# a-to-the-5/Simple-MapReduce-Search-Engine-Information-Retrieval-

Measured on AMD Instinct MI355X. Metric: index build GB/s of text (top-10 queries/sec in 'query'), higher is better.
Workload: dtype u8 text / int32 postings / f64 weights

## Files before the change

simple-mapreduce-search-engine-information-retrieval-_amd/csrc/sme_build.hip:

```cpp
#include <hip/hip_runtime.h>
#include <limits.h>
#include <math.h>
#include <stdio.h>
#include <stdlib.h>
#include <string.h>

#include <algorithm>
#include <memory>
#include <chrono>

#include "sme_internal.hpp"
#include "sme_text.hpp"
#include "sme_trec.hpp"

namespace sme {


template <typename B>
__device__ bool doc_tag_valid(const B &t, int64_t p, const char *tag, int tl) {
  int chain = 0;
  int64_t x = p;
  for (;;) {
    int64_t q = -1;
    for (int j = 1; j < tl; j++) {
// ... 2490 lines not shown
                              uint32_t *ck) {
  for (int64_t i = blockIdx.x * (int64_t)blockDim.x + threadIdx.x; i < P; i += (int64_t)gridDim.x * blockDim.x)
    ck[i] = (key[i] << tfbits) | (tfmask - (uint32_t)tf[i]);
}
__global__ void k_composite32_tf(const uint32_t *ck, int64_t P, uint32_t tfmask, int32_t *tf) {
  for (int64_t i = blockIdx.x * (int64_t)blockDim.x + threadIdx.x; i < P; i += (int64_t)gridDim.x * blockDim.x)
    tf[i] = (int32_t)(tfmask - (ck[i] & tfmask));
}

__global__ void k_term_idf(const int64_t *off, int64_t V, double idf_ref, int64_t N, const int64_t *gdf,
                           const double *idf_by_df, int64_t sdf, const double *idf_by_q, int mode, double *idf) {
  for (int64_t t = blockIdx.x * (int64_t)blockDim.x + threadIdx.x; t < V; t += (int64_t)gridDim.x * blockDim.x) {
    if (mode == SME_IDF_REFERENCE) {
      idf[t] = idf_ref;
    } else {
      const int64_t df = gdf ? gdf[t] : off[t + 1] - off[t];
      idf[t] = df <= sdf ? idf_by_df[df] : idf_by_q[N / df];
    }
  }
}

__global__ void k_composite(const uint32_t *key, const int32_t *tf, int64_t P, int tfbits, uint64_t tfmask,
                            uint64_t *ck) {
  for (int64_t i = blockIdx.x * (int64_t)blockDim.x + threadIdx.x; i < P; i += (int64_t)gridDim.x * blockDim.x)
    ck[i] = ((uint64_t)key[i] << tfbits) | (tfmask - (uint64_t)tf[i]);
}
__global__ void k_composite_tf(const uint64_t *ck, int64_t P, uint64_t tfmask, int32_t *tf) {
  for (int64_t i = blockIdx.x * (int64_t)blockDim.x + threadIdx.x; i < P; i += (int64_t)gridDim.x * blockDim.x)
    tf[i] = (int32_t)(tfmask - (ck[i] & tfmask));
}

__global__ void k_docno_keys(const int32_t *docno, int64_t nR, uint32_t *k, uint32_t *v) {
  for (int64_t i = blockIdx.x * (int64_t)blockDim.x + threadIdx.x; i < nR; i += (int64_t)gridDim.x * blockDim.x) {
    k[i] = (uint32_t)docno[i] ^ 0x80000000u;
    v[i] = (uint32_t)i;
  }
}
__global__ void k_widen_u32(const uint32_t *a, int64_t n, int64_t *b) {
  for (int64_t i = blockIdx.x * (int64_t)blockDim.x + threadIdx.x; i < n; i += (int64_t)gridDim.x * blockDim.x)
    b[i] = (int64_t)a[i];
}
__global__ void k_not_ascending(const int32_t *d, int64_t n, unsigned long long *cnt) {
  bool bad = false;
  for (int64_t i = blockIdx.x * (int64_t)blockDim.x + threadIdx.x + 1; i < n; i += (int64_t)gridDim.x * blockDim.x)
    bad |= d[i] <= d[i - 1];
  if (__any(bad) && (threadIdx.x & 63) == 0) atomicAdd(cnt, 1ull);
}
__global__ void k_iota_i64(int64_t *a, int64_t n) {
  for (int64_t i = blockIdx.x * (int64_t)blockDim.x + threadIdx.x; i < n; i += (int64_t)gridDim.x * blockDim.x) a[i] = i;
}
__global__ void k_adjacent_equal(const uint32_t *k, int64_t n, unsigned long long *cnt) {
  for (int64_t i = blockIdx.x * (int64_t)blockDim.x + threadIdx.x + 1; i < n; i += (int64_t)gridDim.x * blockDim.x)
    if (k[i] == k[i - 1]) atomicAdd(cnt, 1ull);
}
__global__ void k_gather_i64(const int64_t *idx, int64_t n, const int32_t *src, int32_t *dst) {
  for (int64_t i = blockIdx.x * (int64_t)blockDim.x + threadIdx.x; i < n; i += (int64_t)gridDim.x * blockDim.x)
    dst[i] = src[idx[i]];
}
__global__ void k_fill_slow_lens(const int64_t *list, int64_t n, const uint64_t *rs, const uint64_t *re,
                                 int64_t *lens) {
  for (int64_t i = blockIdx.x * (int64_t)blockDim.x + threadIdx.x; i < n; i += (int64_t)gridDim.x * blockDim.x)
    lens[i] = (int64_t)(re[list[i]] - rs[list[i]]) + 1;
}
__global__ void k_compact_flags(const uint8_t *flag, int64_t n, int64_t *list, unsigned long long *cnt) {
  for (int64_t i = blockIdx.x * (int64_t)blockDim.x + threadIdx.x; i < n; i += (int64_t)gridDim.x * blockDim.x)
    if (flag[i]) list[atomicAdd(cnt, 1ull)] = i;
}
__global__ void k_long_lens(const int64_t *list, int64_t n, const int32_t *rlist, const unsigned long long *rep,
                            int64_t *lens) {
  for (int64_t i = blockIdx.x * (int64_t)blockDim.x + threadIdx.x; i < n; i += (int64_t)gridDim.x * blockDim.x) {
    uint32_t len = (uint32_t)(rep[rlist[list[i]]] & 0xFFFFFFull);
    asm volatile("" : "+v"(len));
    lens[i] = 5 * (int64_t)len + 32;
  }
}
__global__ void k_big_list(const int32_t *prec, int64_t n, int64_t *list, unsigned long long *cnt) {
  for (int64_t i = blockIdx.x * (int64_t)blockDim.x + threadIdx.x; i < n; i += (int64_t)gridDim.x * blockDim.x)
    if (prec[i] < 0) list[atomicAdd(cnt, 1ull)] = i;
}
__global__ void k_agg_regions(const int64_t *perm, const int32_t *ntok, int64_t nR, const int32_t *max_nout,
                              int64_t *reg, unsigned long long *mx) {
  unsigned long long m = 0;
  const int64_t mn = max(*max_nout, 1);
  for (int64_t i = blockIdx.x * (int64_t)blockDim.x + threadIdx.x; i < nR; i += (int64_t)gridDim.x * blockDim.x) {
    const int64_t c = (int64_t)ntok[perm[i]] * mn;
    reg[i] = c;
    m = max(m, (unsigned long long)c);
  }
  for (int o = 32; o > 0; o >>= 1) m = max(m, (unsigned long long)__shfl_xor(m, o, 64));
  if ((threadIdx.x & 63) == 0 && m) atomicMax(mx, m);
}
__global__ void k_big_caps(const int64_t *list, int64_t nbig, const int64_t *perm, const int32_t *ntok,
                           const int32_t *max_nout, int64_t *caps) {
  for (int64_t b = blockIdx.x * (int64_t)blockDim.x + threadIdx.x; b < nbig; b += (int64_t)gridDim.x * blockDim.x) {
    int64_t need = (int64_t)ntok[perm[list[b]]] * (int64_t)max(*max_nout, 1) * 2 + 64;
    int64_t c = 1;
    while (c < need) c <<= 1;
    caps[b] = c;
  }
}

__global__ void k_gather_u64(const uint64_t *src, const uint32_t *idx, int64_t nn, uint64_t *dst) {
  for (int64_t i = blockIdx.x * (int64_t)blockDim.x + threadIdx.x; i < nn; i += (int64_t)gridDim.x * blockDim.x)
    dst[i] = src[idx[i]];
}
__global__ void k_iota_u32(uint32_t *a, int64_t nn) {
  for (int64_t i = blockIdx.x * (int64_t)blockDim.x + threadIdx.x; i < nn; i += (int64_t)gridDim.x * blockDim.x)
    a[i] = (uint32_t)i;
}
__global__ void k_pair_counts(const int32_t *prec, const int32_t *bcount, int64_t n, int64_t *out) {
  for (int64_t i = blockIdx.x * (int64_t)blockDim.x + threadIdx.x; i < n; i += (int64_t)gridDim.x * blockDim.x)
    out[i] = prec[i] >= 0 ? prec[i] : bcount[i];
}

constexpr int kGCap = 1024;
constexpr int kGLimit = 768;

__device__ __forceinline__ int32_t nterms_of(const AggIn &in, uint32_t slot) {
  const int32_t rt = in.raw_term[slot];
  return rt >= 0 ? 1 : (rt <= -2 ? in.raw_nout[slot] : 0);
}

__global__ __launch_bounds__(kAggNT) void k_tcount(AggIn in, int64_t nR, int64_t *tcnt) {
  const int wv = threadIdx.x >> 6, lane = threadIdx.x & 63;
  const int64_t nwaves = (int64_t)gridDim.x * (kAggNT / 64);
  for (int64_t i = (int64_t)blockIdx.x * (kAggNT / 64) + wv; i < nR; i += nwaves) {
    const int64_t r = in.perm[i];
    const uint32_t *ts = in.tokstream + (in.rs[r] >> 1);
    const int32_t nt = in.ntok[r];
    int64_t c = 0;
    for (int32_t t = lane; t < nt; t += 64) c += nterms_of(in, ts[t]);
    for (int o = 32; o > 0; o >>= 1) c += __shfl_xor(c, o, 64);
    if (lane == 0) tcnt[i] = c;
  }
}

__global__ __launch_bounds__(kAggNT) void k_twrite(AggIn in, int64_t nR, const int64_t *toff, int32_t *tstream) {
  const int wv = threadIdx.x >> 6, lane = threadIdx.x & 63;
  const int64_t nwaves = (int64_t)gridDim.x * (kAggNT / 64);
  for (int64_t i = (int64_t)blockIdx.x * (kAggNT / 64) + wv; i < nR; i += nwaves) {
    const int64_t r = in.perm[i];
    const uint32_t *ts = in.tokstream + (in.rs[r] >> 1);
    const int32_t nt = in.ntok[r];
    int64_t o = toff[i];
    for (int32_t t0 = 0; t0 < nt; t0 += 64) {
      const int32_t t = t0 + lane;
      const uint32_t slot = t < nt ? ts[t] : 0u;
      const int32_t c = t < nt ? nterms_of(in, slot) : 0;
      const int32_t inc = wave_incl_sum(c);
      const int64_t at = o + inc - c;
      if (c == 1 && in.raw_term[slot] >= 0) {
        tstream[at] = in.raw_term[slot];
      } else if (c > 0) {
        const int32_t m0 = -in.raw_term[slot] - 2;
        for (int32_t m = 0; m < c; m++) tstream[at + m] = in.multi_term[m0 + m];
      }
      o += __shfl(inc, 63, 64);
    }
  }
}

__global__ void k_stream_to_merged(int32_t *tstream, int64_t M, const int64_t *wrank, const int64_t *drank) {
  for (int64_t i = blockIdx.x * (int64_t)blockDim.x + threadIdx.x; i < M; i += (int64_t)gridDim.x * blockDim.x) {
    const int32_t v = tstream[i];
    tstream[i] = (int32_t)((v & kDocCode) ? drank[v & ~kDocCode] : wrank[v]);
  }
}
__global__ void k_stream_docno(const int64_t *perm, const int32_t *docno, int64_t nR, int32_t *out) {
  for (int64_t i = blockIdx.x * (int64_t)blockDim.x + threadIdx.x; i < nR; i += (int64_t)gridDim.x * blockDim.x)
    out[i] = docno[perm[i]];
}

__device__ __forceinline__ uint64_t gram_key(const int32_t *ts, int K, int tb) {
  uint64_t k = 0;
  for (int j = 0; j < K; j++) k = (k << tb) | (uint64_t)(uint32_t)ts[j];
  return k;
}

__device__ __forceinline__ bool gram_insert(uint64_t *keys, int32_t *cnt, uint64_t key, int32_t *distinct) {
  uint32_t h = (uint32_t)fmix64(key) & (kGCap - 1);
  for (int probe = 0; probe < kGCap; probe++) {
    const unsigned long long old = atomicCAS((unsigned long long *)&keys[h], ~0ull, (unsigned long long)key);
    if (old == ~0ull) {
      atomicAdd(distinct, 1);
      atomicAdd(&cnt[h], 1);
      return true;
    }
    if (old == key) {
      atomicAdd(&cnt[h], 1);
      return true;
    }
    h = (h + 1) & (kGCap - 1);
  }
  return false;
}

template <bool EMIT>
__global__ __launch_bounds__(kAggNT) void k_gram_agg(const int32_t *tstream, const int64_t *toff, int64_t nR,
                                                     const int64_t *perm, const int32_t *docno_r, int K, int tb,
                                                     int64_t *pcount, uint8_t *big, const int64_t *pair_off,
                                                     uint64_t *pkey, uint64_t *pval, const uint32_t *pos_key) {
  __shared__ uint64_t keys_all[kAggNT / 64][kGCap];
  __shared__ int32_t cnt_all[kAggNT / 64][kGCap];
  __shared__ int32_t dist_all[kAggNT / 64];
  const int wv = threadIdx.x >> 6, lane = threadIdx.x & 63;
  uint64_t *keys = keys_all[wv];
  int32_t *cnt = cnt_all[wv];
  int32_t *distinct = &dist_all[wv];
  const int64_t nwaves = (int64_t)gridDim.x * (kAggNT / 64);
  for (int64_t i = (int64_t)blockIdx.x * (kAggNT / 64) + wv; i < nR; i += nwaves) {
    const int32_t *ts = tstream + toff[i];
    const int64_t m = toff[i + 1] - toff[i];
    const int64_t ng = m >= K ? m - K + 1 : 0;
    const uint64_t dn = (uint64_t)(uint32_t)docno_r[perm[i]] << 32;
    if (EMIT && big[i]) {
      for (int64_t j = lane; j < ng; j += 64) {
        pkey[pair_off[i] + j] = pos_key ? (uint64_t)pos_key[toff[i] + j] : gram_key(ts + j, K, tb);
        pval[pair_off[i] + j] = dn | 1u;
      }
      continue;
    }
    for (int k = lane; k < kGCap; k += 64) {
      keys[k] = ~0ull;
      cnt[k] = 0;
    }
    if (lane == 0) *distinct = 0;
    wave_sync_lds();
    bool ok = true;
    for (int64_t j = lane; j < ng; j += 64)
      ok &= gram_insert(keys, cnt, pos_key ? (uint64_t)pos_key[toff[i] + j] : gram_key(ts + j, K, tb), distinct);
    wave_sync_lds();
    const int32_t d = *distinct;
    const bool isbig = __any(!ok) || d > kGLimit;
    if (!EMIT) {
      if (lane == 0) {
        pcount[i] = isbig ? ng : d;
        big[i] = isbig;
      }
      wave_sync_lds();
      continue;
    }
    int64_t base = pair_off[i];
    for (int k = 0; k < kGCap / 64; k++) {
      const uint64_t key = keys[k * 64 + lane];
      const uint64_t mb = __ballot(key != ~0ull);
      if (key != ~0ull) {
        const int64_t o = base + __popcll(mb & ((1ull << lane) - 1ull));
        pkey[o] = key;
        pval[o] = dn | (uint32_t)cnt[k * 64 + lane];
      }
      base += __popcll(mb);
    }
    wave_sync_lds();
  }
}

__global__ void k_gram_flags(const uint64_t *k, int64_t P, uint32_t *f) {
  for (int64_t i = blockIdx.x * (int64_t)blockDim.x + threadIdx.x; i < P; i += (int64_t)gridDim.x * blockDim.x)
    f[i] = (i == 0 || k[i] != k[i - 1]) ? 1u : 0u;
}
__global__ void k_gram_ids(const uint64_t *k, const uint32_t *incl, int64_t P, int K, int tb, uint32_t *gid,
                           int32_t *gcomp) {
  for (int64_t i = blockIdx.x * (int64_t)blockDim.x + threadIdx.x; i < P; i += (int64_t)gridDim.x * blockDim.x) {
    const uint32_t g = incl[i] - 1;
    gid[i] = g;
    if (i == 0 || k[i] != k[i - 1])
      for (int j = 0; j < K; j++) gcomp[(int64_t)g * K + j] = (int32_t)((k[i] >> (tb * (K - 1 - j))) & ((1ull << tb) - 1));
  }
}

__global__ __launch_bounds__(kAggNT) void k_gram_round_keys(const int32_t *tstream, const int64_t *toff, int64_t nR,
                                                            int j, int tb, const uint32_t *rprev, uint64_t *key,
                                                            uint32_t *pos) {
  const int wv = threadIdx.x >> 6, lane = threadIdx.x & 63;
  const int64_t nwaves = (int64_t)gridDim.x * (kAggNT / 64);
  for (int64_t i = (int64_t)blockIdx.x * (kAggNT / 64) + wv; i < nR; i += nwaves) {
    const int64_t a = toff[i], e = toff[i + 1];
    for (int64_t p = a + lane; p < e; p += 64) {
      const bool valid = p + j - 1 < e;
      const uint64_t prev = rprev ? (uint64_t)rprev[p] : (uint64_t)(uint32_t)tstream[p];
      key[p] = valid ? (prev << tb) | (uint64_t)(uint32_t)tstream[p + j - 1] : ~0ull;
      pos[p] = (uint32_t)p;
    }
  }
}
__global__ void k_gram_round_heads(const uint64_t *ks, int64_t M, uint32_t *head) {
  for (int64_t s = blockIdx.x * (int64_t)blockDim.x + threadIdx.x; s < M; s += (int64_t)gridDim.x * blockDim.x)
    head[s] = (ks[s] != ~0ull && (s == 0 || ks[s] != ks[s - 1])) ? 1u : 0u;
}
__global__ void k_gram_round_scatter(const uint64_t *ks, const uint32_t *ps, const uint32_t *head,
                                     const uint32_t *excl, int64_t M, uint32_t *rnew, uint32_t *rep) {
  for (int64_t s = blockIdx.x * (int64_t)blockDim.x + threadIdx.x; s < M; s += (int64_t)gridDim.x * blockDim.x) {
    if (ks[s] == ~0ull) continue;
    const uint32_t r = excl[s] + head[s] - 1u;
    rnew[ps[s]] = r;
    if (rep && head[s]) rep[r] = ps[s];
  }
}
__global__ void k_gram_comp_rep(const uint32_t *rep, int64_t Vg, int K, const int32_t *tstream, int32_t *gcomp) {
  for (int64_t g = blockIdx.x * (int64_t)blockDim.x + threadIdx.x; g < Vg; g += (int64_t)gridDim.x * blockDim.x)
    for (int c = 0; c < K; c++) gcomp[g * K + c] = tstream[(int64_t)rep[g] + c];
}

constexpr int kTfTiny = 8;
constexpr int kTfSmall = 64;
constexpr int kTfWave = 512;
constexpr int kTfMedium = 8192;
constexpr int kTfSortMaxTf = 1023;

__global__ __launch_bounds__(256) void k_tfsort_tiny(const int64_t *__restrict__ off, int64_t V,
                                                     const int32_t *__restrict__ docno_d,
                                                     const int32_t *__restrict__ tf_d, int32_t *docno_o,
                                                     int32_t *tf_o) {
  for (int64_t s = blockIdx.x * (int64_t)blockDim.x + threadIdx.x; s < V; s += (int64_t)gridDim.x * blockDim.x) {
    const int64_t b = off[s];
    const int n = (int)(off[s + 1] - b);
    if (n > kTfTiny || n == 0) continue;
    int32_t t[kTfTiny], d[kTfTiny];
#pragma unroll
    for (int j = 0; j < kTfTiny; j++) {
      t[j] = j < n ? tf_d[b + j] : INT_MIN;
      d[j] = j < n ? docno_d[b + j] : 0;
    }
#pragma unroll
    for (int j = 1; j < kTfTiny; j++) {
#pragma unroll
      for (int k = j; k > 0; k--) {
        if (t[k - 1] < t[k]) {
          const int32_t x = t[k - 1], y = d[k - 1];
          t[k - 1] = t[k];
          d[k - 1] = d[k];
          t[k] = x;
          d[k] = y;
        }
      }
    }
#pragma unroll
    for (int j = 0; j < kTfTiny; j++)
      if (j < n) {
        docno_o[b + j] = d[j];
        tf_o[b + j] = t[j];
      }
  }
}

__global__ __launch_bounds__(256) void k_tfsort_small(const int64_t *__restrict__ off,
                                                      const int32_t *__restrict__ seg,
                                                      const unsigned long long *__restrict__ nseg,
                                                      const int32_t *__restrict__ docno_d,
                                                      const int32_t *__restrict__ tf_d, int32_t *docno_o,
                                                      int32_t *tf_o) {
  const int lane = threadIdx.x & 63;
  const int64_t nw = (int64_t)gridDim.x * (blockDim.x >> 6), ns = (int64_t)*nseg;
  for (int64_t q = (int64_t)blockIdx.x * (blockDim.x >> 6) + (threadIdx.x >> 6); q < ns; q += nw) {
    const int64_t s = seg[q];
    const int64_t b = off[s];
    const int n = (int)(off[s + 1] - b);
    const bool v = lane < n;
    const int32_t t = v ? tf_d[b + lane] : 0, d = v ? docno_d[b + lane] : 0;
    int r = 0;
    for (int j = 0; j < n; j++) {
      const int32_t tj = __shfl(t, j, 64);
      r += (tj > t) || (tj == t && j < lane);
    }
    if (v) {
      docno_o[b + r] = d;
      tf_o[b + r] = t;
    }
  }
}

template <int NW>
__global__ __launch_bounds__(NW * 64) void k_tfsort_block(const int64_t *__restrict__ off, int64_t V,
                                                          const int32_t *__restrict__ docno_d,
                                                          const int32_t *__restrict__ tf_d, int32_t *docno_o,
                                                          int32_t *tf_o, const int32_t *__restrict__ seg,
                                                          const unsigned long long *__restrict__ nseg, int max_tf) {
  extern __shared__ int32_t cnt[];
  __shared__ int32_t wsum[NW];
  constexpr int NT = NW * 64;
  const int tid = threadIdx.x, w = tid >> 6, lane = tid & 63;
  const int L = (max_tf + 1) * NW;
  const uint64_t lt_mask = (1ull << lane) - 1;
  const int64_t ns = (int64_t)*nseg;
  for (int64_t q = blockIdx.x; q < ns; q += gridDim.x) {
    const int64_t s = seg[q];
    const int64_t b = off[s], n = off[s + 1] - b;
    for (int j = tid; j < L; j += NT) cnt[j] = 0;
    __syncthreads();
    const int64_t nch = (n + 63) >> 6, cpw = (nch + NW - 1) / NW;
    const int64_t c0 = (int64_t)w * cpw, c1 = c0 + cpw < nch ? c0 + cpw : nch;
    int32_t tn = c0 < c1 && (c0 << 6) + lane < n ? tf_d[b + (c0 << 6) + lane] : -1;
    for (int64_t c = c0; c < c1; c++) {
      const int64_t i = (c << 6) + lane;
      const bool v = i < n;
      const int32_t t = tn;
      tn = c + 1 < c1 && i + 64 < n ? tf_d[b + i + 64] : -1;
      uint64_t pend = __ballot(v);
      while (pend) {
        const int32_t tv = __shfl(t, __ffsll((unsigned long long)pend) - 1, 64);
        const uint64_t m = __ballot(t == tv);
        if (lane == 0) cnt[(max_tf - tv) * NW + w] += __popcll(m);
        pend &= ~m;
      }
    }
    __syncthreads();
    const int per = (L + NT - 1) / NT, j0 = tid * per, j1 = j0 + per < L ? j0 + per : L;
    int run = 0;
    for (int j = j0; j < j1; j++) run += cnt[j];
    int inc = run;
#pragma unroll
    for (int o = 1; o < 64; o <<= 1) {
      const int u = __shfl_up(inc, o, 64);
      if (lane >= o) inc += u;
    }
    if (lane == 63) wsum[w] = inc;
    __syncthreads();
    int base = inc - run;
    for (int k = 0; k < w; k++) base += wsum[k];
    for (int j = j0; j < j1; j++) {
      const int c = cnt[j];
      cnt[j] = base;
      base += c;
    }
    __syncthreads();
    int32_t tn2 = -1, dn2 = 0;
    if (c0 < c1 && (c0 << 6) + lane < n) {
      tn2 = tf_d[b + (c0 << 6) + lane];
      dn2 = docno_d[b + (c0 << 6) + lane];
    }
    for (int64_t c = c0; c < c1; c++) {
      const int64_t i = (c << 6) + lane;
      const bool v = i < n;
      const int32_t t = tn2, d = dn2;
      if (c + 1 < c1 && i + 64 < n) {
        tn2 = tf_d[b + i + 64];
        dn2 = docno_d[b + i + 64];
      } else {
        tn2 = -1;
      }
      uint64_t pend = __ballot(v);
      while (pend) {
        const int32_t tv = __shfl(t, __ffsll((unsigned long long)pend) - 1, 64);
        const uint64_t m = __ballot(t == tv);
        const int slot = (max_tf - tv) * NW + w;
        const int cb = cnt[slot];
        if (t == tv) {
          const int64_t p = b + cb + __popcll(m & lt_mask);
          docno_o[p] = d;
          tf_o[p] = t;
        }
        if (lane == 0) cnt[slot] = cb + __popcll(m);
        pend &= ~m;
      }
    }
    __syncthreads();
  }
}

constexpr int kTfTile = 4096;

__global__ __launch_bounds__(256) void k_tf_classify(const int64_t *__restrict__ off, int64_t V, int32_t *med,
                                                     int32_t *large, int32_t *small, int32_t *wave,
                                                     unsigned long long *ctr) {
  __shared__ unsigned int s_n[4];
  __shared__ unsigned long long s_b[4];
  for (int64_t s0 = (int64_t)blockIdx.x * 256; s0 < V; s0 += (int64_t)gridDim.x * 256) {
    const int64_t s = s0 + threadIdx.x;
    const int64_t n = s < V ? off[s + 1] - off[s] : 0;
    const int cls = n > kTfMedium ? 1 : n > kTfWave ? 0 : n > kTfSmall ? 3 : n > kTfTiny ? 2 : -1;
    if (threadIdx.x < 4) s_n[threadIdx.x] = 0;
    __syncthreads();
    unsigned int pos = 0;
    if (cls >= 0) pos = atomicAdd(&s_n[cls], 1u);
    __syncthreads();
    if (threadIdx.x < 4)
      s_b[threadIdx.x] = s_n[threadIdx.x] ? atomicAdd(&ctr[threadIdx.x], (unsigned long long)s_n[threadIdx.x]) : 0ull;
    __syncthreads();
    if (cls == 0) med[s_b[0] + pos] = (int32_t)s;
    if (cls == 1) large[s_b[1] + pos] = (int32_t)s;
    if (cls == 2) small[s_b[2] + pos] = (int32_t)s;
    if (cls == 3) wave[s_b[3] + pos] = (int32_t)s;
    __syncthreads();
  }
}
__global__ void k_tf_ntiles(const int64_t *off, const int32_t *large, const unsigned long long *nlarge, int64_t V,
                            int64_t *nt) {
  const int64_t nl = (int64_t)*nlarge;
  for (int64_t q = blockIdx.x * (int64_t)blockDim.x + threadIdx.x; q <= V; q += (int64_t)gridDim.x * blockDim.x) {
    const int64_t n = q < nl ? off[large[q] + 1] - off[large[q]] : 0;
    nt[q] = (n + kTfTile - 1) / kTfTile;
  }
}

__device__ __forceinline__ int64_t tile_segment(const int64_t *toff, int64_t V, int64_t tau) {
  int64_t lo = 0, hi = V;
  while (hi - lo > 1) {
    const int64_t mid = (lo + hi) >> 1;
    if (toff[mid] <= tau) lo = mid;
    else hi = mid;
  }
  return lo;
}

__global__ __launch_bounds__(256) void k_tf_tile_count(const int64_t *__restrict__ off,
                                                       const int32_t *__restrict__ large,
                                                       const unsigned long long *__restrict__ nlarge,
                                                       const int64_t *__restrict__ toff, int64_t ntiles,
                                                       const int32_t *__restrict__ tf_d, int max_tf,
                                                       int32_t *tcnt) {
  extern __shared__ int32_t h[];
  const int w = threadIdx.x >> 6, lane = threadIdx.x & 63, F = max_tf + 1;
  int32_t *hw = h + w * F;
  const int64_t nwv = (int64_t)gridDim.x * 4;
  const int64_t nl = (int64_t)*nlarge;
  for (int64_t tau = (int64_t)blockIdx.x * 4 + w; tau < ntiles; tau += nwv) {
    const int64_t q = tile_segment(toff, nl, tau), s = large[q];
    const int64_t b = off[s] + (tau - toff[q]) * kTfTile, e = min(off[s + 1], b + (int64_t)kTfTile);
    for (int j = lane; j < F; j += 64) hw[j] = 0;
    __builtin_amdgcn_wave_barrier();
    int32_t tn = b + lane < e ? tf_d[b + lane] : -1;
    for (int64_t c = b; c < e; c += 64) {
      const bool v = c + lane < e;
      const int32_t t = tn;
      tn = c + 64 + lane < e ? tf_d[c + 64 + lane] : -1;
      uint64_t pend = __ballot(v);
      while (pend) {
        const int32_t tv = __shfl(t, __ffsll((unsigned long long)pend) - 1, 64);
        const uint64_t m = __ballot(t == tv);
        if (lane == 0) hw[max_tf - tv] += __popcll(m);
        pend &= ~m;
      }
    }
    __builtin_amdgcn_wave_barrier();
    for (int j = lane; j < F; j += 64) tcnt[tau * F + j] = hw[j];
    __builtin_amdgcn_wave_barrier();
  }
}

__global__ __launch_bounds__(256) void k_tf_tile_scan(const unsigned long long *__restrict__ nlarge,
                                                      const int64_t *__restrict__ toff, int max_tf, int32_t *tcnt) {
  __shared__ int32_t sc[256 / 64 + 1];
  const int tid = threadIdx.x, F = max_tf + 1;
  const int64_t nl = (int64_t)*nlarge;
  for (int64_t q = blockIdx.x; q < nl; q += gridDim.x) {
    const int64_t t0 = toff[q], T = toff[q + 1] - t0;
    int32_t *c = tcnt + t0 * F;
    int32_t carry = 0;
    for (int f0 = 0; f0 < F; f0 += 256) {
      const int f = f0 + tid;
      int32_t tot = 0;
      if (f < F) {
#pragma unroll 8
        for (int64_t j = 0; j < T; j++) tot += c[j * F + f];
      }
      int32_t all;
      int32_t run = carry + block_excl_sum<256, int32_t>(tot, sc, &all);
      carry += all;
      if (f < F) {
#pragma unroll 8
        for (int64_t j = 0; j < T; j++) {
          const int32_t x = c[j * F + f];
          c[j * F + f] = run;
          run += x;
        }
      }
    }
  }
}

__global__ __launch_bounds__(256) void k_tf_tile_place(const int64_t *__restrict__ off,
                                                       const int32_t *__restrict__ large,
                                                       const unsigned long long *__restrict__ nlarge,
                                                       const int64_t *__restrict__ toff, int64_t ntiles,
                                                       const int32_t *__restrict__ docno_d,
                                                       const int32_t *__restrict__ tf_d, int max_tf,
                                                       const int32_t *__restrict__ tcnt, int32_t *docno_o,
                                                       int32_t *tf_o) {
  extern __shared__ int32_t h[];
  const int w = threadIdx.x >> 6, lane = threadIdx.x & 63, F = max_tf + 1;
  int32_t *hw = h + w * F;
  const uint64_t lt_mask = (1ull << lane) - 1;
  const int64_t nwv = (int64_t)gridDim.x * 4;
  const int64_t nl = (int64_t)*nlarge;
  for (int64_t tau = (int64_t)blockIdx.x * 4 + w; tau < ntiles; tau += nwv) {
    const int64_t q = tile_segment(toff, nl, tau), s = large[q];
    const int64_t sb = off[s];
    const int64_t b = sb + (tau - toff[q]) * kTfTile, e = min(off[s + 1], b + (int64_t)kTfTile);
    for (int j = lane; j < F; j += 64) hw[j] = tcnt[tau * F + j];
    __builtin_amdgcn_wave_barrier();
    int32_t tn = b + lane < e ? tf_d[b + lane] : -1, dnx = b + lane < e ? docno_d[b + lane] : 0;
    for (int64_t c = b; c < e; c += 64) {
      const bool v = c + lane < e;
      const int32_t t = tn, d = dnx;
      const int64_t in = c + 64 + lane;
      tn = in < e ? tf_d[in] : -1;
      dnx = in < e ? docno_d[in] : 0;
      uint64_t pend = __ballot(v);
      while (pend) {
        const int32_t tv = __shfl(t, __ffsll((unsigned long long)pend) - 1, 64);
        const uint64_t m = __ballot(t == tv);
        const int slot = max_tf - tv;
        const int cb = hw[slot];
        if (t == tv) {
          const int64_t p = sb + cb + __popcll(m & lt_mask);
          docno_o[p] = d;
          tf_o[p] = t;
        }
        if (lane == 0) hw[slot] = cb + __popcll(m);
        pend &= ~m;
      }
    }
    __builtin_amdgcn_wave_barrier();
  }
}

static int grid_for(int64_t n, int nt = 256, int cap = 8192) {
  int64_t g = (n + nt - 1) / nt;
  if (g < 1) g = 1;
  if (g > cap) g = cap;
  return (int)g;
}

template <typename T>
static T d2h(const T *d, hipStream_t st) {
  T h;
#if SME_D2H_PINNED
  static thread_local void *pin = nullptr;
  if (!pin) SME_HIP(hipHostMalloc(&pin, 64, hipHostMallocDefault));
  static_assert(sizeof(T) <= 64, "d2h");
  SME_HIP(hipMemcpyAsync(pin, d, sizeof(T), hipMemcpyDeviceToHost, st));
  SME_HIP(hipStreamSynchronize(st));
  memcpy(&h, pin, sizeof(T));
#else
  SME_HIP(hipMemcpyAsync(&h, d, sizeof(T), hipMemcpyDeviceToHost, st));
  SME_HIP(hipStreamSynchronize(st));
#endif
  return h;
}

static int bits_for(uint64_t v) {
  int b = 0;
  while (b < 64 && (1ull << b) <= v) b++;
  return b < 1 ? 1 : b;
}

enum {
  W_S, W_E, W_C, W_CNT, W_EOF, W_NEXTS, W_RS, W_RE, W_DOCNO, W_SLOW, W_SLOWLIST, W_SCROFF, W_U16, W_BOFF,
  W_TOK, W_NTOK, W_RKEYS, W_RREPS, W_POOL, W_CKEY, W_CSTR, W_NOUT, W_LONG, W_FKEYS, W_FREPS, W_CFINAL,
  W_VSLOT, W_KHI, W_KLO, W_VIDX, W_T0, W_T1, W_T2, W_T3, W_RAWTERM, W_MULTI, W_PERM, W_PREC, W_PTERM, W_PVAL,
  W_MAXNOUT, W_SS, W_SE, W_SC, W_RLIST, W_RFLAG, W_POFF, W_OVFKEY, W_FREC, W_LT, W_RADIX, W_NTOK2, W_BIGL2,
  W_BIGCAP, W_SEGB, W_VCS, W_DMARK, W_DSLOT, W_DLIST, W_DSRC, W_DKEY, W_WRANK, W_DSPAN, W_RLISTW,
  W_NSLOTS
};
constexpr int kBuildWs = 64;
static_assert(W_NSLOTS <= 64, "too many build workspace slots");

RecordSpans find_records(sme_ctx *cx, const uint8_t *t, uint64_t n, hipStream_t st, Prof *prof) {
  DevBuf *W = cx->ws + kBuildWs;
  auto cub_tmp = [&](size_t bytes) { return cx->cub_tmp.get(bytes); };
  unsigned long long *cnt = W[W_CNT].as<unsigned long long>(16);
  uint64_t capL = std::max<uint64_t>(cx->lt_cap_hint, std::max<uint64_t>(4096, n / 256));
  uint64_t *ltpos = nullptr;
  int64_t nlt = 0;
  int lt_attempts = 0;
  for (int attempt = 0;; attempt++) {
    lt_attempts++;
    ltpos = W[W_LT].as<uint64_t>(capL);
    SME_HIP(hipMemsetAsync(cnt, 0, 16 * sizeof(unsigned long long), st));
    hipLaunchKernelGGL(k_scan_lt, dim3(grid_for((int64_t)ceil_div(n, 64), 256, 4096)), dim3(kScanNT), 0, st, t,
                       (int64_t)n, ltpos, capL, cnt + 3);
    SME_CHECK_LAUNCH();
    nlt = (int64_t)d2h(cnt + 3, st);
    if ((uint64_t)nlt <= capL) break;
    if (attempt > 2) throw Error(SME_ELIMIT, "'<' list capacity");
    capL = (uint64_t)nlt + 1024;
  }
  cx->lt_cap_hint = std::max<uint64_t>(cx->lt_cap_hint, (uint64_t)nlt + (uint64_t)nlt / 8 + 1024);
  uint64_t capS = std::max<uint64_t>(1024, (uint64_t)nlt + 1), capE = capS, capC = capS;
  unsigned long long h_cnt[3];
  for (int attempt = 0;; attempt++) {
    ScanOut so;
    so.S = W[W_S].as<uint64_t>(capS);
    so.E = W[W_E].as<uint64_t>(capE);
    so.C = W[W_C].as<uint64_t>(capC);
    so.capS = (uint32_t)std::min<uint64_t>(capS, 0xFFFFFFFFu);
    so.capE = (uint32_t)std::min<uint64_t>(capE, 0xFFFFFFFFu);
    so.capC = (uint32_t)std::min<uint64_t>(capC, 0xFFFFFFFFu);
    so.cnt = cnt;
    SME_HIP(hipMemsetAsync(cnt, 0, 3 * sizeof(unsigned long long), st));
    if (nlt > 0)
      hipLaunchKernelGGL(k_tag_classify, dim3(grid_for(nlt, 256, 8192)), dim3(kScanNT), 0, st, t, (int64_t)n, ltpos,
                         nlt, so);
    SME_CHECK_LAUNCH();
    SME_HIP(hipMemcpyAsync(h_cnt, cnt, sizeof h_cnt, hipMemcpyDeviceToHost, st));
    SME_HIP(hipStreamSynchronize(st));
    if (h_cnt[0] <= capS && h_cnt[1] <= capE && h_cnt[2] <= capC) break;
    if (attempt > 2) throw Error(SME_ELIMIT, "tag scan capacity");
    capS = std::max<uint64_t>(capS, h_cnt[0]);
    capE = std::max<uint64_t>(capE, h_cnt[1]);
    capC = std::max<uint64_t>(capC, h_cnt[2]);
  }
  const int64_t nS = (int64_t)h_cnt[0], nE = (int64_t)h_cnt[1], nC = (int64_t)h_cnt[2];
  if (prof) prof->mark("scan_tags");

  auto sort_u64 = [&](uint64_t *buf, int64_t cnt_, int slot_alt) -> uint64_t * {
    if (cnt_ < 2) return buf;
    uint64_t *alt = W[slot_alt].as<uint64_t>(cnt_);
    uint32_t *va = cx->ws[26].as<uint32_t>(cnt_), *vb = cx->ws[27].as<uint32_t>(cnt_);
    uint32_t *rscr = cx->ws[24].as<uint32_t>(kv_sort_scratch(cnt_) / sizeof(uint32_t) + 1);
    return kv_sort<uint64_t>(buf, va, alt, vb, cnt_, bits_for(n), rscr, st, true) == va ? buf : alt;
  };
  uint64_t *S = sort_u64(W[W_S].as<uint64_t>(capS), nS, W_SS);
  uint64_t *E = sort_u64(W[W_E].as<uint64_t>(capE), nE, W_SE);
  uint64_t *C = sort_u64(W[W_C].as<uint64_t>(capC), nC, W_SC);

  int64_t *e_of = W[W_EOF].as<int64_t>(nS + 1), *next_s = W[W_NEXTS].as<int64_t>(nS + 1);
  SME_HIP(hipMemsetAsync(cnt, 0, 16 * sizeof(unsigned long long), st));
  int64_t nR = 0;
  uint64_t *rs = W[W_RS].as<uint64_t>(nS + 1), *re = W[W_RE].as<uint64_t>(nS + 1);
  if (nS > 0) {
    hipLaunchKernelGGL(k_chain, dim3(grid_for(nS)), dim3(256), 0, st, S, nS, E, nE, e_of, next_s, cnt);
    SME_CHECK_LAUNCH();
    unsigned long long hc[3];
    SME_HIP(hipMemcpyAsync(hc, cnt, sizeof hc, hipMemcpyDeviceToHost, st));
    SME_HIP(hipStreamSynchronize(st));
    const unsigned long long bad = hc[0];
    if (bad == 0) {
      nR = (int64_t)hc[2];
      if (nR > 0)
        hipLaunchKernelGGL(k_records_direct, dim3(grid_for(nR)), dim3(256), 0, st, S, E, e_of, nR, rs, re);
    } else {
      hipLaunchKernelGGL(k_records_walk, dim3(1), dim3(64), 0, st, S, nS, E, e_of, next_s, rs, re, cnt + 1);
      SME_CHECK_LAUNCH();
      nR = (int64_t)d2h(cnt + 1, st);
    }
  }
  if (prof) prof->mark("records");
  return RecordSpans{rs, re, nR, C, nC, lt_attempts};
}

__global__ void k_iota_docno(int32_t *d, int64_t n) {
  for (int64_t i = blockIdx.x * (int64_t)blockDim.x + threadIdx.x; i < n; i += (int64_t)gridDim.x * blockDim.x)
    d[i] = (int32_t)(i + 1);
}

void build_docid_hash(sme_ctx *cx, bool distinct, hipStream_t st) {
  cx->map_hash_ok = false;
  if (!distinct || cx->map_n < 2) return;
  const uint64_t cap = next_pow2(std::max<uint64_t>(1024, 2 * (uint64_t)cx->map_n));
  uint32_t *slots = cx->map_slots.as<uint32_t>(cap);
  unsigned int *ovf = cx->ws[63].as<unsigned int>(4);
  SME_HIP(hipMemsetAsync(slots, 0, cap * sizeof(uint32_t), st));
  SME_HIP(hipMemsetAsync(ovf, 0, sizeof(unsigned int), st));
  hipLaunchKernelGGL(k_map_hash, dim3(grid_for(cx->map_n)), dim3(256), 0, st, (const uint16_t *)cx->map_chars.p,
                     (const int64_t *)cx->map_off.p, cx->map_n, slots, cap - 1, ovf);
  SME_CHECK_LAUNCH();
  cx->map_mask = cap - 1;
  cx->map_hash_ok = d2h(ovf, st) == 0;
}

sme_index *build_index(sme_ctx *cx, const uint8_t *t, uint64_t n, hipStream_t st, int job) {
  if (job == 0 && !cx->has_map) throw Error(SME_ENOMAP, "no docno mapping loaded (sme_load_docno_mapping)");
  DevBuf *W = cx->ws + kBuildWs;
  Prof prof(st, &cx->prof_events);
  auto cub_tmp = [&](size_t bytes) { return cx->cub_tmp.get(bytes); };
  unsigned long long *cnt = W[W_CNT].as<unsigned long long>(40);

  uint8_t early_code[128];
  const RecordSpans rsp = find_records(cx, t, n, st, &prof);
  uint64_t *rs = rsp.rs, *re = rsp.re, *C = rsp.C;
  const int64_t nR = rsp.nR, nC = rsp.nC;

  int32_t *docno = W[W_DOCNO].as<int32_t>(nR + 1);
  uint64_t *dspan = job == 0 ? W[W_DSPAN].as<uint64_t>(nR + 1) : nullptr;
  SME_HIP(hipMemsetAsync(cnt, 0, 16 * sizeof(unsigned long long), st));
  if (nR > 0 && job == 0) {
    hipLaunchKernelGGL(k_docno, dim3(grid_for(nR)), dim3(256), 0, st, t, (int64_t)n, rs, re, nR,
                       (const uint16_t *)cx->map_chars.p, (const int64_t *)cx->map_off.p, cx->map_n,
                       cx->map_hash_ok ? (const uint32_t *)cx->map_slots.p : nullptr, cx->map_mask, docno, cnt,
                       dspan);
    SME_CHECK_LAUNCH();
  } else if (nR > 0) {
    hipLaunchKernelGGL(k_iota_docno, dim3(grid_for(nR)), dim3(256), 0, st, docno, nR);
  }
  uint8_t *slow = W[W_SLOW].as<uint8_t>(nR + 1);
  int32_t *frec = W[W_FREC].as<int32_t>(nR + 1);
  if (nR > 0) {
    hipLaunchKernelGGL(k_mark_slow, dim3(grid_for(nR)), dim3(256), 0, st, rs, re, nR, C, nC, slow, cnt + 1);
    hipLaunchKernelGGL(k_not_ascending, dim3(grid_for(nR)), dim3(256), 0, st, docno, nR, cnt + 3);
    uint8_t *fflag = W[W_RFLAG].as<uint8_t>(nR);
    hipLaunchKernelGGL(k_not_flags, dim3(grid_for(nR)), dim3(256), 0, st, slow, nR, fflag);
    select_flagged(fflag, nR, frec, reinterpret_cast<int32_t *>(cnt + 14), cx->ws[25], cx->ws[23], st);
    SME_CHECK_LAUNCH();
  }
  unsigned long long h2[16];
  SME_HIP(hipMemcpyAsync(h2, cnt, sizeof h2, hipMemcpyDeviceToHost, st));
  SME_HIP(hipStreamSynchronize(st));
  if (h2[0]) throw Error(SME_EPARSE, "a record has <DOCNO> but no </DOCNO> (TrecDocument.getDocid throws)");
  const int64_t nslow = (int64_t)h2[1];
  const int64_t nF = nR > 0 ? (int64_t)(int32_t)(uint32_t)h2[14] : 0;
  prof.mark("docno");

  int64_t *perm = W[W_PERM].as<int64_t>(nR + 1);
  bool dup_docno = false;
  bool ascending = false;
  if (nR > 0) {
    ascending = h2[3] == 0;
    if (ascending) hipLaunchKernelGGL(k_iota_i64, dim3(grid_for(nR)), dim3(256), 0, st, perm, nR);
  }
  if (nR > 0 && !ascending) {
    uint32_t *k0 = W[W_T0].as<uint32_t>(nR), *k1 = W[W_T1].as<uint32_t>(nR);
    uint32_t *v0 = W[W_T2].as<uint32_t>(nR), *v1 = W[W_T3].as<uint32_t>(nR);
    hipLaunchKernelGGL(k_docno_keys, dim3(grid_for(nR)), dim3(256), 0, st, docno, nR, k0, v0);
    uint32_t *rscr = cx->ws[24].as<uint32_t>(kv_sort_scratch(nR) / sizeof(uint32_t) + 1);
    uint32_t *vs = kv_sort<uint32_t>(k0, v0, k1, v1, nR, 32, rscr, st, true);
    const uint32_t *ks = vs == v0 ? k0 : k1;
    hipLaunchKernelGGL(k_widen_u32, dim3(grid_for(nR)), dim3(256), 0, st, vs, nR, perm);
    SME_HIP(hipMemsetAsync(cnt, 0, 16 * sizeof(unsigned long long), st));
    hipLaunchKernelGGL(k_adjacent_equal, dim3(grid_for(nR)), dim3(256), 0, st, ks, nR, cnt);
    dup_docno = d2h(cnt, st) != 0;
  }
  prof.mark("docno_sort");

  uint64_t rcap = cx->raw_cap_hint
                      ? cx->raw_cap_hint
                      : next_pow2(std::max<uint64_t>(1ull << 20, std::min<uint64_t>(n / 256, 1ull << 30)));
  uint32_t *tok = W[W_TOK].as<uint32_t>(n / 2 + 2);
  int32_t *ntok = W[W_NTOK].as<int32_t>(nR + 1);
  RawTable tb;
  unsigned int *ovf = reinterpret_cast<unsigned int *>(cnt + 8);
  int64_t h_nsel = 0;
  int tok_attempts = 0, vocab_attempts = 0;

  for (int attempt = 0;; attempt++) {
    tok_attempts++;
    {
      uint8_t *rb = W[W_RKEYS].as<uint8_t>(rcap * kRawSlotBytes);
      tb.tok = reinterpret_cast<ulonglong2 *>(rb);
      tb.key = reinterpret_cast<unsigned long long *>(rb + rcap * sizeof(ulonglong2));
      tb.rep = tb.key + rcap;
    }
    tb.mask = rcap - 1;
    tb.text = t;
    tb.overflow = ovf;
    SME_HIP(hipMemsetAsync(tb.tok, 0, rcap * kRawSlotBytes, st));
    SME_HIP(hipMemsetAsync(cnt, 0, 16 * sizeof(unsigned long long), st));
    if (nR > 0) {
      if (nF > 0) {
        uint64_t *rsF = W[W_LT].as<uint64_t>(2 * (size_t)nF), *reF = rsF + nF;
        hipLaunchKernelGGL(k_gather_bounds, dim3(grid_for(nF)), dim3(256), 0, st, frec, nF, rs, re, rsF, reF);
        prof.mark("tok_setup");
        const int64_t tgrid = std::max<int64_t>(1, std::min<int64_t>(nF, cx->opt_tok_grid)),
                      rpb = (nF + tgrid - 1) / tgrid;
        int tokexp = 0;
#ifdef SME_EXPERIMENTS
        if (const char *tx = getenv("SME_TOKEXP")) tokexp = atoi(tx);
#endif
        hipLaunchKernelGGL(k_tok_fast, dim3((unsigned)((nF + rpb - 1) / rpb)), dim3(kTokNT), 0, st, t, (int64_t)n, rsF,
                           reF, frec, nF, rpb, tok, ntok, tb, tokexp);
        SME_CHECK_LAUNCH();
        prof.mark("tok_kernel");
      }
    }
    if (nslow > 0) {
      int64_t *slist = W[W_SLOWLIST].as<int64_t>(nslow);
      hipLaunchKernelGGL(k_compact_flags, dim3(grid_for(nR)), dim3(256), 0, st, slow, nR, slist, cnt + 2);
      int64_t *lens = W[W_T0].as<int64_t>(nslow + 1), *soff = W[W_SCROFF].as<int64_t>(nslow + 1);
      hipLaunchKernelGGL(k_fill_slow_lens, dim3(grid_for(nslow)), dim3(256), 0, st, slist, nslow, rs, re, lens);
      size_t tbb = 0;
      SME_HIP(hipMemsetAsync(lens + nslow, 0, sizeof(int64_t), st));
      excl_scan(lens, soff, (int64_t)(nslow + 1), cx->ws[23], st);
      int64_t tot = d2h(soff + nslow, st);
      uint16_t *u16s = W[W_U16].as<uint16_t>(tot + 1);
      uint32_t *boffs = W[W_BOFF].as<uint32_t>(tot + 1);
      hipLaunchKernelGGL(k_tok_slow, dim3(grid_for(nslow, 64)), dim3(64), 0, st, t, rs, re, slist, nslow, soff,
                         u16s, boffs, tok, ntok, tb);
      SME_CHECK_LAUNCH();
    }
    hipLaunchKernelGGL(k_raw_flags, dim3(grid_for((int64_t)rcap)), dim3(256), 0, st, tb.key, rcap,
                       W[W_RFLAG].as<uint8_t>(rcap));
    select_flagged(W[W_RFLAG].as<uint8_t>(rcap), (int64_t)rcap, W[W_RLIST].as<int32_t>(rcap),
                   reinterpret_cast<int32_t *>(cnt + 13), cx->ws[25], cx->ws[23], st);
    unsigned long long hov[6];
    SME_HIP(hipMemcpyAsync(hov, cnt + 8, sizeof hov, hipMemcpyDeviceToHost, st));
    SME_HIP(hipStreamSynchronize(st));
    const unsigned int of = (unsigned int)hov[0];
    h_nsel = (int64_t)(int32_t)(uint32_t)hov[5];
    if (of == 0) break;
    if (of & 2u) throw Error(SME_ELIMIT, "a raw token is longer than 16 MiB");
    if (attempt > 3 || rcap >= (1ull << 32)) throw Error(SME_ELIMIT, "raw vocabulary table overflow");
    rcap <<= 2;
  }
  prof.mark("tokenize");

  int32_t *const rlist_all = W[W_RLIST].as<int32_t>(rcap);
  const int64_t nraw_all = h_nsel;
  {
    const uint64_t pct = (uint64_t)std::max<int64_t>(10, std::min<int64_t>(90, cx->opt_raw_load_pct));
    cx->raw_cap_hint = next_pow2(std::max<uint64_t>(1ull << 20, (uint64_t)nraw_all * 100 / pct + 1));
  }
  bool dfast = cx->opt_docid_terms != 0 && nR > 0 && nraw_all > 0 && dspan != nullptr;
  int32_t *rlist_w = nullptr;
  int64_t nraw_w = 0;
  uint32_t *dmark = nullptr;
  int32_t *dslot = nullptr, *dl = nullptr;
  uint64_t *dsrc = nullptr;
  Key16 *dkey = nullptr;
  int64_t Vd = 0;
  if (dfast) {
    unsigned long long *dcnt = reinterpret_cast<unsigned long long *>(W[W_DSRC].as<uint64_t>(4));
    dmark = W[W_DMARK].as<uint32_t>(rcap);
    dslot = W[W_DSLOT].as<int32_t>(nR + 1);
    SME_HIP(hipMemsetAsync(dmark, 0xFF, rcap * sizeof(uint32_t), st));
    hipLaunchKernelGGL(k_docid_slots, dim3(grid_for(nR)), dim3(256), 0, st, t, (int64_t)n, dspan, nR, tb, dslot,
                       dmark);
    uint8_t *dflag = reinterpret_cast<uint8_t *>(W[W_DKEY].as<Key16>(nR / 16 + 1));
    hipLaunchKernelGGL(k_docid_flags, dim3(grid_for(nR)), dim3(256), 0, st, dslot, nR, dflag);
// ... 477 lines not shown
      ai.dmin = h_drange[0];
      ai.F = (uint32_t)Fq;
    }
  }
  if (!ai.v32) p_val = W[W_PVAL].as<uint64_t>(P + 1);
  if (nR > 0) {
    hipLaunchKernelGGL(k_agg_w<true>, dim3(agg_grid), dim3(kAggNT), 0, st, ai, nR, prec, pair_off, p_term, p_val);
    SME_CHECK_LAUNCH();
  }
  if (nbig > 0) {
    hipLaunchKernelGGL(k_agg_big, dim3((unsigned)std::min<int64_t>(nbig, 4096)), dim3(kAggNT), 0, st, ai, big_list,
                       nbig, boff, bcap, gkeys, gcnt, bcount, pair_off, p_term, p_val, 1);
    SME_CHECK_LAUNCH();
  }
  } else if (K >= 2) {
    const int tb = bits_for((uint64_t)std::max<int64_t>(V, 1));
    const bool ranked = (int64_t)K * tb > 63 || cx->opt_kgram_rank;
    const unsigned g_grid = (unsigned)std::min<int64_t>(std::max<int64_t>((nR + 3) / 4, 1), 8192);
    int64_t *tcnt = W[W_T2].as<int64_t>(nR + 1), *toff = W[W_T3].as<int64_t>(nR + 1);
    if (nR > 0) hipLaunchKernelGGL(k_tcount, dim3(g_grid), dim3(kAggNT), 0, st, ai, nR, tcnt);
    SME_HIP(hipMemsetAsync(tcnt + nR, 0, sizeof(int64_t), st));
    size_t tbb = 0;
    excl_scan(tcnt, toff, (int64_t)(nR + 1), cx->ws[23], st);
    const int64_t M = d2h(toff + nR, st);
    int32_t *tstream = W[W_U16].as<int32_t>(M + 1);
    if (nR > 0) hipLaunchKernelGGL(k_twrite, dim3(g_grid), dim3(kAggNT), 0, st, ai, nR, toff, tstream);
    const uint32_t *pos_key = nullptr;
    const uint32_t *grep = nullptr;
    int64_t Vr = 0;
    if (ranked && M > 0) {
      if (M > 0xFFFFFFFFll) throw Error(SME_ELIMIT, "k-gram ranking of more than 2^32 term positions");
      uint64_t *ka = W[W_FKEYS].as<uint64_t>(M + 1), *kb = W[W_OVFKEY].as<uint64_t>(M + 1);
      uint32_t *pa = W[W_FREPS].as<uint32_t>(M + 1), *pb = W[W_RREPS].as<uint32_t>(M + 1);
      uint32_t *ra = W[W_RKEYS].as<uint32_t>(M + 1), *rb = W[W_CSTR].as<uint32_t>(M + 1);
      uint32_t *head = W[W_RLIST].as<uint32_t>(M + 2), *excl = W[W_POFF].as<uint32_t>(M + 2);
      uint32_t *rep = W[W_SEGB].as<uint32_t>(M + 1);
      uint32_t *rscr = W[W_RADIX].as<uint32_t>(kv_sort_scratch(M) / sizeof(uint32_t) + 1);
      const uint32_t *rprev = nullptr;
      int64_t nprev = V;
      for (int j = 2; j <= K; j++) {
        hipLaunchKernelGGL(k_gram_round_keys, dim3(g_grid), dim3(kAggNT), 0, st, tstream, toff, nR, j, tb, rprev, ka,
                           pa);
        const int kbits = std::min(64, bits_for((uint64_t)std::max<int64_t>(nprev, 1)) + tb + 1);
        uint32_t *ps = kv_sort<uint64_t>(ka, pa, kb, pb, M, kbits, rscr, st, true);
        const uint64_t *ks = ps == pa ? ka : kb;
        hipLaunchKernelGGL(k_gram_round_heads, dim3(grid_for(M)), dim3(256), 0, st, ks, M, head);
        SME_HIP(hipMemsetAsync(head + M, 0, sizeof(uint32_t), st));
        excl_scan(head, excl, M + 1, cx->ws[23], st);
        uint32_t *rnew = (rprev == ra) ? rb : ra;
        hipLaunchKernelGGL(k_gram_round_scatter, dim3(grid_for(M)), dim3(256), 0, st, ks, ps, head, excl, M, rnew,
                           j == K ? rep : nullptr);
        SME_CHECK_LAUNCH();
        nprev = (int64_t)d2h(excl + M, st);
        rprev = rnew;
      }
      pos_key = rprev;
      grep = rep;
      Vr = nprev;
    }
    int64_t *pcount = W[W_T1].as<int64_t>(nR + 1), *pair_off = W[W_T0].as<int64_t>(nR + 1);
    uint8_t *bigf = W[W_SLOW].as<uint8_t>(nR + 1);
    if (nR > 0)
      hipLaunchKernelGGL(k_gram_agg<false>, dim3(g_grid), dim3(kAggNT), 0, st, tstream, toff, nR, perm, docno, K, tb,
                         pcount, bigf, nullptr, nullptr, nullptr, pos_key);
    SME_HIP(hipMemsetAsync(pcount + nR, 0, sizeof(int64_t), st));
    excl_scan(pcount, pair_off, (int64_t)(nR + 1), cx->ws[23], st);
    const int64_t Pg = d2h(pair_off + nR, st);
    uint64_t *pkey = W[W_KHI].as<uint64_t>(Pg + 1), *pval0 = W[W_KLO].as<uint64_t>(Pg + 1);
    if (nR > 0)
      hipLaunchKernelGGL(k_gram_agg<true>, dim3(g_grid), dim3(kAggNT), 0, st, tstream, toff, nR, perm, docno, K, tb,
                         pcount, bigf, pair_off, pkey, pval0, pos_key);
    SME_CHECK_LAUNCH();
    uint64_t *pkey_s = W[W_CKEY].as<uint64_t>(Pg + 1);
    p_val = W[W_PVAL].as<uint64_t>(Pg + 1);
    if (Pg > 0) {
      sort_pairs_v64<uint64_t>(pkey, pkey_s, pval0, p_val, Pg,
                               ranked ? bits_for((uint64_t)std::max<int64_t>(Vr, 1)) : K * tb, cx->ws[120],
                               cx->ws[121], cx->ws[122], st);
    }
    uint32_t *gflag = W[W_VSLOT].as<uint32_t>(Pg + 1), *gincl = W[W_VIDX].as<uint32_t>(Pg + 2);
    p_term = W[W_PTERM].as<uint32_t>(Pg + 1);
    int64_t Vg = 0;
    if (Pg > 0) {
      hipLaunchKernelGGL(k_gram_flags, dim3(grid_for(Pg)), dim3(256), 0, st, pkey_s, Pg, gflag);
      SME_HIP(hipMemsetAsync(gflag + Pg, 0, sizeof(uint32_t), st));
      excl_scan(gflag, gincl, Pg + 1, cx->ws[23], st);
      gincl += 1;
      Vg = (int64_t)d2h(gincl + Pg - 1, st);
      int32_t *gcomp = ix->d_gram.as<int32_t>(Vg * K + 1);
      hipLaunchKernelGGL(k_gram_ids, dim3(grid_for(Pg)), dim3(256), 0, st, pkey_s, gincl, Pg, ranked ? 0 : K, tb,
                         p_term, gcomp);
      if (ranked)
        hipLaunchKernelGGL(k_gram_comp_rep, dim3(grid_for(Vg)), dim3(256), 0, st, grep, Vg, K, tstream, gcomp);
      SME_CHECK_LAUNCH();
    } else {
      ix->d_gram.get(16);
    }
    P = Pg;
      Vi = Vg;
    ix->P = P;
    dup_docno = true;
  }
  prof.mark("aggregate");

  if (K == 1 && cx->opt_positions) {
    DevBuf tcb;
    tcb.pool = &cx->pool;
    const unsigned g_grid = (unsigned)std::min<int64_t>(std::max<int64_t>((nR + 3) / 4, 1), 8192);
    int64_t *tcnt = tcb.as<int64_t>(nR + 1), *toff = ix->d_ps_off.as<int64_t>(nR + 1);
    if (nR > 0) hipLaunchKernelGGL(k_tcount, dim3(g_grid), dim3(kAggNT), 0, st, ai, nR, tcnt);
    SME_HIP(hipMemsetAsync(tcnt + nR, 0, sizeof(int64_t), st));
    excl_scan(tcnt, toff, (int64_t)(nR + 1), cx->ws[23], st);
    const int64_t M = d2h(toff + nR, st);
    if (M >= (int64_t(1) << 31)) throw Error(SME_ELIMIT, "positions: 2^31 or more term positions");
    int32_t *tstream = ix->d_ps_terms.as<int32_t>(M + 1);
    int32_t *pdn = ix->d_ps_docno.as<int32_t>(nR + 1);
    if (nR > 0) {
      hipLaunchKernelGGL(k_twrite, dim3(g_grid), dim3(kAggNT), 0, st, ai, nR, toff, tstream);
      if (dsplit && M > 0)
        hipLaunchKernelGGL(k_stream_to_merged, dim3(grid_for(M)), dim3(256), 0, st, tstream, M,
                           (const int64_t *)wrank_all, (const int64_t *)drank);
      hipLaunchKernelGGL(k_stream_docno, dim3(grid_for(nR)), dim3(256), 0, st, (const int64_t *)perm,
                         (const int32_t *)docno, nR, pdn);
    }
    SME_CHECK_LAUNCH();
    SME_HIP(hipStreamSynchronize(st));
    ix->ps_records = nR;
    ix->ps_terms = M;
    ix->has_positions = true;
    prof.mark("positions");
  }

  const bool split = dsplit && ai.dk_rec != nullptr;
  int64_t Pw = P, Nd = 0;
  uint32_t *dk = nullptr, *dv = nullptr;
  uint2 *xw = nullptr;
  if (split) {
    uint8_t *dfl = W[W_RREPS].as<uint8_t>(nR + 1);
    int32_t *didx = W[W_CFINAL].as<int32_t>(nR + 1);
    hipLaunchKernelGGL(k_dsplit_flags, dim3(grid_for(nR)), dim3(256), 0, st, ai.dk_rec, nR, dfl);
    SME_HIP(hipMemsetAsync(cnt + 33, 0, 2 * sizeof(unsigned long long), st));
    select_flagged(dfl, nR, didx, reinterpret_cast<int32_t *>(cnt + 33), cx->ws[25], cx->ws[23], st);
    dk = W[W_CSTR].as<uint32_t>(nR + 1);
    dv = W[W_VIDX].as<uint32_t>(nR + 1);
    hipLaunchKernelGGL(k_dsplit_gather, dim3(grid_for(nR)), dim3(256), 0, st, didx, cnt + 33, ai.dk_rec, ai.dv_rec, dk,
                       dv, cnt + 34);
    SME_CHECK_LAUNCH();
    unsigned long long hd[2];
    SME_HIP(hipMemcpyAsync(hd, cnt + 33, sizeof hd, hipMemcpyDeviceToHost, st));
    SME_HIP(hipStreamSynchronize(st));
    Nd = (int64_t)(uint32_t)hd[0];
    if (hd[1] != 0 && Nd > 1) {
      uint32_t *dk2 = W[W_LONG].as<uint32_t>(Nd + 1), *dv2 = reinterpret_cast<uint32_t *>(W[W_OVFKEY].as<uint64_t>(Nd / 2 + 1));
      uint32_t *rs2 = W[W_RADIX].as<uint32_t>(kv_sort_scratch(Nd) / sizeof(uint32_t) + 1);
      if (kv_sort<uint32_t>(dk, dv, dk2, dv2, Nd, bits_for((uint64_t)Vd), rs2, st, true) != dv) {
        dk = dk2;
        dv = dv2;
      }
    }
    xw = reinterpret_cast<uint2 *>(W[W_DKEY].as<Key16>(Vw / 2 + 1));
    if (Vw > 0)
      hipLaunchKernelGGL(k_word_shift, dim3(grid_for(Vw)), dim3(256), 0, st, (const int64_t *)wrank_all, Vw, dk, Nd,
                         xw);
    SME_CHECK_LAUNCH();
    P = Pw + Nd;
    if (P > 0xFFFFFFFFll) throw Error(SME_ELIMIT, "term sort of more than 2^32 pairs");
    ix->P = P;
    prof.mark("docid_pairs");
  }
  const int tbits = split ? bits_for((uint64_t)std::max<int64_t>(Vw - 1, 1)) : bits_for((uint64_t)std::max<int64_t>(Vi, 1));
  uint32_t *key_s = W[W_T0].as<uint32_t>(P + 1);
  int64_t Pm = P;
  int32_t max_tf = 1;
  bool packed = false;
  int64_t dmin = 0;
  uint32_t F = 0;
  if (ai.v32 != nullptr || ai.rec_val != nullptr) {
    max_tf = std::max<int32_t>(1, h_mtf);
    packed = true;
    dmin = ai.dmin;
    F = ai.F;
  } else if (P > 0 && !dup_docno && K == 1) {
    SME_HIP(hipMemsetAsync(mtf, 0, sizeof(unsigned int), st));
    const int h_init[2] = {INT_MAX, INT_MIN};
    SME_HIP(hipMemcpyAsync(dmn, h_init, sizeof h_init, hipMemcpyHostToDevice, st));
    hipLaunchKernelGGL(k_pair_stats, dim3(grid_for(P, 256, 2048)), dim3(256), 0, st, p_val, P, mtf);
    hipLaunchKernelGGL(k_docno_range, dim3(grid_for(nR, 256, 1024)), dim3(256), 0, st, docno, nR, dmn, dmx);
    unsigned int h_m = d2h(mtf, st);
    int h_r[2];
    SME_HIP(hipMemcpyAsync(h_r, dmn, sizeof h_r, hipMemcpyDeviceToHost, st));
    SME_HIP(hipStreamSynchronize(st));
    const uint64_t Fq = (uint64_t)h_m + 1, D = (uint64_t)((int64_t)h_r[1] - (int64_t)h_r[0] + 1);
    max_tf = std::max<int32_t>(1, (int32_t)h_m);
    packed = D * Fq < (1ull << 32) && tbits + bits_for((uint64_t)max_tf) <= 32;
    dmin = h_r[0];
    F = (uint32_t)Fq;
  }
  int32_t *docno_d = nullptr, *tf_d = nullptr;
  int64_t *off = nullptr;
  std::vector<double> early_lut;
  bool weights_fused = false;
  if (packed) {
    const int sort_bits = cx->opt_sort_bits > 0 ? (int)cx->opt_sort_bits : (Pw > (int64_t(1) << 30) ? 8 : 11);
    uint32_t *v32 = ai.v32;
    if (ai.rec_val != nullptr) {
      if (term_sort_passes(tbits, sort_bits) >= 3) v32 = W[W_PVAL].as<uint32_t>(P + 1);
    } else if (v32 == nullptr) {
      v32 = reinterpret_cast<uint32_t *>(W[W_T1].as<uint64_t>(P + 1));
      hipLaunchKernelGGL(k_pack_pairs, dim3(grid_for(P)), dim3(256), 0, st, p_val, P, dmin, F, v32);
    }
    uint32_t *v32s = W[W_T2].as<uint32_t>(P + 1);
    docno_d = ix->d_docno_d.as<int32_t>(P + 1);
    tf_d = ix->d_tf_d.as<int32_t>(P + 1);
    uint32_t *rscr = W[W_RADIX].as<uint32_t>(term_sort_scratch(P) / sizeof(uint32_t) + 1);
    double *wf = nullptr;
    if (ix->idf_mode == SME_IDF_REFERENCE && P > 0) {
      early_lut.assign((size_t)max_tf + 1, 0.0);
      for (int i = 1; i <= max_tf; i++) early_lut[(size_t)i] = 1.0 + log((double)i);
      SME_HIP(hipMemcpyAsync(ix->d_lut.as<double>(max_tf + 1), early_lut.data(), early_lut.size() * sizeof(double),
                             hipMemcpyHostToDevice, st));
      wf = ix->d_w.as<double>(P + 1);
      weights_fused = true;
    }
    const double idf_r = log10((double)(std::max<int64_t>(nR, 0) / 1));
    key_s = term_sort(p_term, v32, key_s, v32s, sort_nrec, sort_reg, sort_xoff, Pw, tbits, dmin, F, docno_d, tf_d, rscr,
                      st, wf ? (const double *)ix->d_lut.p : nullptr, idf_r, wf, sort_bits, xw, P, ai.rec_val,
                      ai.tf_shift);
    off = ix->d_off.as<int64_t>(Vi + 1);
    SME_HIP(hipMemsetAsync(off, 0, (Vi + 1) * sizeof(int64_t), st));
    if (!split) {
      hipLaunchKernelGGL(k_term_offsets<false>, dim3(grid_for(P)), dim3(256), 0, st, key_s, P, off, Vi);
    } else {
      hipLaunchKernelGGL(k_term_offsets<true>, dim3(grid_for(P)), dim3(256), 0, st, key_s, P, off, Vi);
      hipLaunchKernelGGL(k_docid_off, dim3(grid_for(Vd)), dim3(256), 0, st, dk, Nd, Vd, (const int64_t *)drank,
                         (const int64_t *)wrank_all, Vw, xw, Pw, off);
      if (Nd > 0)
        hipLaunchKernelGGL(k_docid_place, dim3(grid_for(Nd)), dim3(256), 0, st, dk, dv, Nd, (const int64_t *)drank,
                           (const int64_t *)wrank_all, Vw, xw, off, Pw, dmin, F, docno_d, tf_d, key_s,
                           wf ? (const double *)ix->d_lut.p : nullptr, idf_r, wf);
    }
    SME_CHECK_LAUNCH();
  } else {
    uint64_t *val_s = W[W_T1].as<uint64_t>(P + 1);
    if (P > 0)
      sort_pairs_v64<uint32_t>(p_term, key_s, p_val, val_s, P, tbits, cx->ws[120], cx->ws[121], cx->ws[122], st);
    if (dup_docno && P > 0) {
      uint64_t *ck = W[W_PVAL].as<uint64_t>(P), *ck2 = W[W_T2].as<uint64_t>(P);
      int32_t *tfv = reinterpret_cast<int32_t *>(W[W_PTERM].as<uint32_t>(P)), *tf2 = W[W_T3].as<int32_t>(P);
      hipLaunchKernelGGL(k_dup_keys, dim3(grid_for(P)), dim3(256), 0, st, key_s, val_s, P, ck, tfv);
      int64_t *nout = reinterpret_cast<int64_t *>(cnt + 10);
      reduce_by_key_sum(ck, tfv, P, ck2, tf2, nout, cx->ws[120], cx->ws[121], cx->ws[23], st);
      Pm = d2h(nout, st);
      hipLaunchKernelGGL(k_dup_unpack, dim3(grid_for(Pm)), dim3(256), 0, st, ck2, tf2, Pm, key_s, val_s);
    }
    off = ix->d_off.as<int64_t>(Vi + 1);
    SME_HIP(hipMemsetAsync(off, 0, (Vi + 1) * sizeof(int64_t), st));
    if (Pm > 0) hipLaunchKernelGGL(k_term_offsets<false>, dim3(grid_for(Pm)), dim3(256), 0, st, key_s, Pm, off, Vi);
    docno_d = ix->d_docno_d.as<int32_t>(Pm + 1);
    tf_d = ix->d_tf_d.as<int32_t>(Pm + 1);
    if (Pm > 0) hipLaunchKernelGGL(k_unpack_vals, dim3(grid_for(Pm)), dim3(256), 0, st, val_s, Pm, docno_d, tf_d);
    SME_CHECK_LAUNCH();
    if (Pm > 0) {
      int32_t *mx = reinterpret_cast<int32_t *>(cnt + 11);
      reduce_max<int32_t>(tf_d, Pm, mx, st);
      max_tf = std::max(1, d2h(mx, st));
    }
  }
  ix->P = Pm;
  const int64_t PP = Pm;
  prof.mark("sort_term");

  ix->max_tf = max_tf;
  {
    std::vector<double> lut(max_tf + 1, 0.0);
    for (int i = 1; i <= max_tf; i++) lut[i] = 1.0 + log((double)i);
    double *d_lut = ix->d_lut.as<double>(max_tf + 1);
    SME_HIP(hipMemcpyAsync(d_lut, lut.data(), lut.size() * sizeof(double), hipMemcpyHostToDevice, st));
    const int64_t Nn = std::max<int64_t>(nR, 0);
    ix->idf_N = Nn;
    double idf_ref = idf_value(Nn, 1);
    int64_t sdf = (int64_t)std::sqrt((double)std::max<int64_t>(Nn, 1)) + 1;
    std::vector<double> by_df(sdf + 1), by_q(Nn / std::max<int64_t>(sdf, 1) + 2);
    for (int64_t d = 1; d <= sdf; d++) by_df[d] = idf_value(Nn, d);
    for (size_t q = 0; q < by_q.size(); q++) by_q[q] = idf_value((int64_t)q, 1);
    double *d_bydf = W[W_U16].as<double>(by_df.size() + by_q.size());
    double *d_byq = d_bydf + by_df.size();
    SME_HIP(hipMemcpyAsync(d_bydf, by_df.data(), by_df.size() * sizeof(double), hipMemcpyHostToDevice, st));
    SME_HIP(hipMemcpyAsync(d_byq, by_q.data(), by_q.size() * sizeof(double), hipMemcpyHostToDevice, st));
    double *idf = ix->d_idf.as<double>(Vi + 1);
    if (Vi > 0)
      hipLaunchKernelGGL(k_term_idf, dim3(grid_for(Vi)), dim3(256), 0, st, off, Vi, idf_ref, Nn, nullptr, d_bydf, sdf,
                         d_byq, ix->idf_mode, idf);
    double *w = ix->d_w.as<double>(PP + 1);
    if (PP > 0 && !weights_fused)
      hipLaunchKernelGGL(k_weights, dim3(grid_for(PP)), dim3(256), 0, st, key_s, tf_d, PP, d_lut, idf_ref, off, Nn,
                         d_bydf, sdf, d_byq, ix->idf_mode, w);
    SME_CHECK_LAUNCH();
    SME_HIP(hipStreamSynchronize(st));
  }
  prof.mark("weights");

  int32_t *docno_o = ix->d_docno_o.as<int32_t>(PP + 1), *tf_o = ix->d_tf_o.as<int32_t>(PP + 1);
  if (PP > 0 && max_tf <= kTfSortMaxTf) {
    hipLaunchKernelGGL(k_tfsort_tiny, dim3(grid_for(Vi)), dim3(256), 0, st, off, Vi, docno_d, tf_d, docno_o, tf_o);
    int64_t *ntl = W[W_FKEYS].as<int64_t>(3 * (Vi + 1)), *toff = W[W_FREPS].as<int64_t>(Vi + 1);
    int32_t *seg_med = reinterpret_cast<int32_t *>(ntl + Vi + 1), *seg_large = seg_med + Vi,
            *seg_small = seg_large + Vi, *seg_wave = seg_small + Vi;
    unsigned long long *nseg = cnt + 28;
    SME_HIP(hipMemsetAsync(nseg, 0, 4 * sizeof(unsigned long long), st));
    hipLaunchKernelGGL(k_tf_classify, dim3(grid_for(Vi)), dim3(256), 0, st, off, Vi, seg_med, seg_large, seg_small,
                       seg_wave, nseg);
    hipStream_t s2 = cx->aux_stream;
    SME_HIP(hipEventRecord(cx->ev_fork, st));
    SME_HIP(hipStreamWaitEvent(s2, cx->ev_fork, 0));
    struct AuxJoin {
      hipStream_t st, s2;
      hipEvent_t ev;
      ~AuxJoin() {
        (void)hipEventRecord(ev, s2);
        (void)hipStreamWaitEvent(st, ev, 0);
      }
    } aux_join{st, s2, cx->ev_join};
    hipLaunchKernelGGL(k_tfsort_small, dim3(grid_for(Vi * 64, 256, 8192)), dim3(256), 0, s2, off, seg_small, nseg + 2,
                       docno_d, tf_d, docno_o, tf_o);
    const size_t lds4 = (size_t)(max_tf + 1) * 4 * sizeof(int32_t);
    hipLaunchKernelGGL(k_tfsort_block<4>, dim3((unsigned)std::min<int64_t>(std::max<int64_t>(Vi, 1), 4096)),
                       dim3(256), lds4, s2, off, Vi, docno_d, tf_d, docno_o, tf_o, seg_med, nseg, max_tf);
    hipLaunchKernelGGL(k_tfsort_block<1>, dim3((unsigned)std::min<int64_t>(std::max<int64_t>(Vi, 1), 32768)),
                       dim3(64), lds4 / 4, s2, off, Vi, docno_d, tf_d, docno_o, tf_o, seg_wave, nseg + 3, max_tf);
    SME_CHECK_LAUNCH();
    hipLaunchKernelGGL(k_tf_ntiles, dim3(grid_for(Vi + 1)), dim3(256), 0, st, off, seg_large, nseg + 1, Vi, ntl);
    size_t tbb = 0;
    excl_scan(ntl, toff, (int64_t)(Vi + 1), cx->ws[23], st);
    const int64_t ntiles = d2h(toff + Vi, st);
    if (ntiles > 0) {
      const int F = max_tf + 1;
      int32_t *tcnt = reinterpret_cast<int32_t *>(W[W_CKEY].as<uint64_t>((ntiles * F + 1) / 2 + 1));
      const unsigned tg = (unsigned)std::min<int64_t>((ntiles + 3) / 4, 8192);
      hipLaunchKernelGGL(k_tf_tile_count, dim3(tg), dim3(256), (size_t)4 * F * sizeof(int32_t), st, off, seg_large,
                         nseg + 1, toff, ntiles, tf_d, max_tf, tcnt);
      hipLaunchKernelGGL(k_tf_tile_scan, dim3((unsigned)std::min<int64_t>(Vi, 8192)), dim3(256), 0, st, nseg + 1,
                         toff, max_tf, tcnt);
      hipLaunchKernelGGL(k_tf_tile_place, dim3(tg), dim3(256), (size_t)4 * F * sizeof(int32_t), st, off, seg_large,
                         nseg + 1, toff, ntiles, docno_d, tf_d, max_tf, tcnt, docno_o, tf_o);
    }
    SME_CHECK_LAUNCH();
  } else if (PP > 0) {
    const int tfb = bits_for((uint64_t)max_tf);
    const int kbits = bits_for((uint64_t)std::max<int64_t>(Vi, 1));
    if (kbits + tfb <= 32) {
      const uint32_t tfmask = (uint32_t)((1ull << tfb) - 1);
      uint32_t *ck = reinterpret_cast<uint32_t *>(W[W_PVAL].as<uint64_t>(PP)), *ck2 = W[W_T2].as<uint32_t>(PP);
      hipLaunchKernelGGL(k_composite32, dim3(grid_for(PP)), dim3(256), 0, st, key_s, tf_d, PP, tfb, tfmask, ck);
      uint32_t *dv = W[W_T3].as<uint32_t>(PP);
      SME_HIP(hipMemcpyAsync(dv, docno_d, (size_t)PP * sizeof(int32_t), hipMemcpyDeviceToDevice, st));
      sort_pairs<uint32_t>(ck, ck2, dv, reinterpret_cast<uint32_t *>(docno_o), PP, kbits + tfb, cx->ws[122], st);
      hipLaunchKernelGGL(k_composite32_tf, dim3(grid_for(PP)), dim3(256), 0, st, ck2, PP, tfmask, tf_o);
    } else {
      const uint64_t tfmask = (1ull << tfb) - 1;
      uint64_t *ck = W[W_PVAL].as<uint64_t>(PP), *ck2 = W[W_T2].as<uint64_t>(PP);
      hipLaunchKernelGGL(k_composite, dim3(grid_for(PP)), dim3(256), 0, st, key_s, tf_d, PP, tfb, tfmask, ck);
      uint32_t *dv = W[W_T3].as<uint32_t>(PP);
      SME_HIP(hipMemcpyAsync(dv, docno_d, (size_t)PP * sizeof(int32_t), hipMemcpyDeviceToDevice, st));
      sort_pairs<uint64_t>(ck, ck2, dv, reinterpret_cast<uint32_t *>(docno_o), PP, kbits + tfb, cx->ws[122], st);
      hipLaunchKernelGGL(k_composite_tf, dim3(grid_for(PP)), dim3(256), 0, st, ck2, PP, tfmask, tf_o);
    }
    SME_CHECK_LAUNCH();
  }
  prof.mark("sort_tf");

  int32_t *rdn = ix->d_rec_docno.as<int32_t>(nR + 1);
  if (nR > 0 && want_packed && h_drange[1] >= h_drange[0]) {
    SME_HIP(hipMemcpyAsync(rdn, docno, nR * sizeof(int32_t), hipMemcpyDeviceToDevice, st));
    ix->dmin = h_drange[0];
    ix->dmax = h_drange[1];
  } else if (nR > 0) {
    SME_HIP(hipMemcpyAsync(rdn, docno, nR * sizeof(int32_t), hipMemcpyDeviceToDevice, st));
    int *dmn = reinterpret_cast<int *>(cnt + 12), *dmx = dmn + 1;
    const int h_init[2] = {INT_MAX, INT_MIN};
    SME_HIP(hipMemcpyAsync(dmn, h_init, sizeof h_init, hipMemcpyHostToDevice, st));
    hipLaunchKernelGGL(k_docno_range, dim3(grid_for(nR, 256, 1024)), dim3(256), 0, st, docno, nR, dmn, dmx);
    int h_r[2];
    SME_HIP(hipMemcpyAsync(h_r, dmn, sizeof h_r, hipMemcpyDeviceToHost, st));
    SME_HIP(hipStreamSynchronize(st));
    ix->dmin = h_r[0];
    ix->dmax = h_r[1];
  }
  prof.mark("finalize");
  ix->V = Vi;
  ix->Vt = V;
  ix->profile = prof.finish();
  ix->profile.emplace_back("tok_attempts", (float)tok_attempts);
  ix->profile.emplace_back("records_fast", (float)nF);
  ix->profile.emplace_back("records_slow", (float)nslow);
  ix->profile.emplace_back("vocab_attempts", (float)vocab_attempts);
  ix->profile.emplace_back("lt_attempts", (float)rsp.lt_attempts);
  ix_guard.release();
  return ix;
}

__global__ void k_reweight(const int64_t *off, int64_t V, const int32_t *tf, const double *lut, double idf_ref,
                           const int64_t *gdf, int64_t N, const double *idf_by_df, int64_t sdf, const double *idf_by_q,
                           int mode, double *w) {
  const int lane = threadIdx.x & 63;
  const int64_t wpb = blockDim.x / 64;
  for (int64_t t = blockIdx.x * wpb + (threadIdx.x >> 6); t < V; t += (int64_t)gridDim.x * wpb) {
    double idf = idf_ref;
    if (mode != SME_IDF_REFERENCE) {
      int64_t df = gdf ? gdf[t] : off[t + 1] - off[t];
      idf = df <= sdf ? idf_by_df[df] : idf_by_q[N / df];
    }
    for (int64_t p = off[t] + lane; p < off[t + 1]; p += 64) w[p] = __dmul_rn(lut[tf[p]], idf);
  }
}

__global__ void k_reweight_flat(const uint32_t *term_of, const int32_t *tf, int64_t P, const double *lut,
                                const double *idf, double *w) {
  for (int64_t p = blockIdx.x * (int64_t)blockDim.x + threadIdx.x; p < P; p += (int64_t)gridDim.x * blockDim.x)
    w[p] = __dmul_rn(lut[tf[p]], idf[term_of[p]]);
}

void reweight_index(sme_index *ix, int64_t N, const int64_t *d_gdf, hipStream_t st, const uint32_t *d_term_of) {
  auto &W = ix->ctx->ws;
  std::vector<double> lut(ix->max_tf + 1, 0.0);
  for (int i = 1; i <= ix->max_tf; i++) lut[i] = 1.0 + log((double)i);
  const int64_t Nn = std::max<int64_t>(N, 0);
  ix->idf_N = Nn;
  double idf_ref = idf_value(Nn, 1);
  int64_t sdf = (int64_t)std::sqrt((double)std::max<int64_t>(Nn, 1)) + 1;
  std::vector<double> by_df(sdf + 1), by_q(Nn / std::max<int64_t>(sdf, 1) + 2);
  for (int64_t d = 1; d <= sdf; d++) by_df[d] = idf_value(Nn, d);
  for (size_t q = 0; q < by_q.size(); q++) by_q[q] = idf_value((int64_t)q, 1);
  double *d_lut = ix->d_lut.as<double>(lut.size());
  double *d_tab = W[57].as<double>(by_df.size() + by_q.size());
  SME_HIP(hipMemcpyAsync(d_lut, lut.data(), lut.size() * sizeof(double), hipMemcpyHostToDevice, st));
  SME_HIP(hipMemcpyAsync(d_tab, by_df.data(), by_df.size() * sizeof(double), hipMemcpyHostToDevice, st));
  SME_HIP(hipMemcpyAsync(d_tab + by_df.size(), by_q.data(), by_q.size() * sizeof(double), hipMemcpyHostToDevice, st));
  if (ix->V > 0)
    hipLaunchKernelGGL(k_term_idf, dim3((unsigned)std::min<int64_t>((ix->V + 255) / 256, 65536)), dim3(256), 0, st,
                       (const int64_t *)ix->d_off.p, ix->V, idf_ref, Nn, d_gdf, d_tab, sdf, d_tab + by_df.size(),
                       ix->idf_mode, (double *)ix->d_idf.p);
  if (ix->V > 0 && d_term_of && ix->P > 0)
    hipLaunchKernelGGL(k_reweight_flat, dim3((unsigned)std::min<int64_t>((ix->P + 255) / 256, 65536)), dim3(256), 0, st,
                       d_term_of, (const int32_t *)ix->d_tf_d.p, ix->P, d_lut, (const double *)ix->d_idf.p,
                       (double *)ix->d_w.p);
  else if (ix->V > 0)
    hipLaunchKernelGGL(k_reweight, dim3((unsigned)std::min<int64_t>((ix->V + 3) / 4, 65536)),
                       dim3(256), 0, st, (const int64_t *)ix->d_off.p, ix->V, (const int32_t *)ix->d_tf_d.p, d_lut,
                       idf_ref, d_gdf, Nn, d_tab, sdf, d_tab + by_df.size(), ix->idf_mode, (double *)ix->d_w.p);
  SME_CHECK_LAUNCH();
  SME_HIP(hipStreamSynchronize(st));
  ix->q_ready = false;
}

}
```

simple-mapreduce-search-engine-information-retrieval-_amd/csrc/sme_internal.hpp:

```cpp
#pragma once
#include <hip/hip_runtime.h>
#include <math.h>
#include <stdint.h>

#include <memory>
#include <string>
#include <vector>

#include "sme_common.hpp"

struct sme_ctx {
  sme::BufPool pool;
  sme_config cfg{};
  int device = 0;
  hipStream_t own_stream = nullptr;
  hipStream_t aux_stream = nullptr;
  hipEvent_t ev_fork = nullptr, ev_join = nullptr;
  std::vector<hipEvent_t> prof_events;
  sme::DevBuf map_chars, map_off;
  int64_t map_n = 0;
  bool has_map = false;
  sme::DevBuf map_slots;
  uint64_t map_mask = 0;
  bool map_hash_ok = false;
  sme::DevBuf ws[128];
  sme::DevBuf cub_tmp;
  sme::DevBuf q_gates;
  uint64_t vocab_long_cap = 0, vocab_ovf_cap = 0, raw_cap_hint = 0, lt_cap_hint = 0;
  std::string profile_json;
  std::vector<std::pair<std::string, float>> last_profile;
  std::vector<uint8_t> mapping_out;
  std::vector<int32_t> h_wlist;
  float last_query_ms = -1.0f;
  float last_query_prep_ms = -1.0f;
  float last_query_index_ms = -1.0f;
  bool last_query_tiled = false;
  const char *last_query_name = "k_query";
  float last_query_seed_ms = 0.0f, last_query_final_ms = 0.0f, last_query_total_ms = 0.0f;
  int64_t last_query_overflow = 0;
  int64_t last_query_fallback = 0;
  int64_t last_query_stages = 0;
  int64_t last_query_slices = 0;
  bool last_query_split = false;
  int64_t opt_query_kernel = 0;
  int64_t opt_heavy_div = 128;
  int64_t opt_seed_tiles = 4;
  int64_t opt_query_order = 1;
  int64_t opt_agg_two_pass = 0;
  int64_t opt_agg_grid = 0;
  int64_t opt_tok_grid = 5120;
  int64_t opt_raw_load_pct = 40;
  int64_t opt_docid_terms = 1;
  int64_t opt_sort_bits = 0;
  int64_t opt_docid_split = 1;
  int64_t opt_cand_cap = 1024;
  int64_t opt_seed_m = 64;
  int64_t opt_kgram_rank = 0;
  int64_t opt_win_slice = 0;
  int64_t opt_win_sample = 1;
  int64_t opt_win_stage_min = 0;
  int64_t opt_query_budget = 0;
  int64_t opt_wild_scan = 0;
  int64_t opt_wild_chunk = 1024;
  int64_t opt_fuzzy_scan = 0;
  int64_t opt_bool_chunk = 1024;
  int64_t opt_bool_driver = 0;
  int64_t opt_positions = 0;
  int64_t opt_corpus_keep = int64_t(16) << 30;
  void *h_stage[2] = {nullptr, nullptr};
  size_t h_stage_cap = 0;
  sme::DevBuf h_corpus_dev;
  int live_indexes = 0;
  bool destroyed = false;
};

struct sme_index {
  sme_ctx *ctx = nullptr;
  int K = 1, R = 1, idf_mode = 0;
  int job = 0;
  int64_t cg_ngrams = 0, cg_pairs = 0;
  int64_t N = 0, V = 0, P = 0;
  int64_t Vt = 0;
  int32_t max_tf = 0;
  int64_t dmin = 0, dmax = -1;
  sme::DevBuf d_term_off;
  sme::DevBuf d_term_chars;
  sme::DevBuf d_off;
  sme::DevBuf d_docno_d;
  sme::DevBuf d_tf_d;
  sme::DevBuf d_w;
  sme::DevBuf d_idf;
  sme::DevBuf d_gram;
  sme::DevBuf d_lut;
  sme::DevBuf d_docno_o;
  sme::DevBuf d_tf_o;
  sme::DevBuf d_rec_docno;
  sme::DevBuf d_rec_first;
  bool records_only = false;
  bool from_records = false;
  sme::DevBuf d_ser;
  std::vector<int64_t> part_start;
  bool ser_ready = false;
  float ser_ms = 0.0f;
  std::vector<std::unique_ptr<uint8_t[]>> h_parts;
  std::vector<char> h_parts_ready;
  std::vector<int64_t> h_off;
  std::vector<int32_t> h_docno, h_tf, h_df;
  bool h_csr_ready = false;
  std::vector<int64_t> h_term_off;
  std::vector<uint16_t> h_term_chars;
  std::vector<int32_t> h_gram;
  std::vector<uint8_t> h_term_tmp;
  bool h_terms_ready = false;
  sme::DevBuf d_hrow_of;
  sme::DevBuf d_heavy;
  const uint8_t *q_tfrow = nullptr, *q_bm16 = nullptr, *q_bm1k = nullptr, *q_imp = nullptr;
  const uint8_t *q_sbq = nullptr;
  sme::DevBuf d_spk;
  const uint32_t *q_spk = nullptr;
  double q_alpha = 1.0;
  unsigned long long q_wmax_bits = 0;
  int64_t q_T = 0, q_H = 0, q_div = -1;
  bool q_ready = false;
  float q_prep_ms = 0.0f;
  sme::DevBuf d_wkeys;
  sme::DevBuf d_wgoff;
  sme::DevBuf d_wgterm;
  int64_t wild_G = 0, wild_pairs = 0;
  bool wild_ready = false;
  float wild_ms = 0.0f;
  sme::DevBuf d_wx_off;
  sme::DevBuf d_wx_ids;
  sme::DevBuf d_wx_in, d_wx_plan, d_wx_choff, d_wx_moff, d_wx_scan;
  int64_t wx_total = 0;
  std::vector<int64_t> h_wx_off;
  std::vector<int32_t> h_wx_ids;
  sme::DevBuf d_fz_off;
  sme::DevBuf d_fz_ids;
  sme::DevBuf d_fz_dist;
  int64_t fz_total = 0;
  uint64_t fz_scanned = 0, fz_cands = 0;
  std::vector<int64_t> h_fz_off;
  std::vector<int32_t> h_fz_ids;
  std::vector<uint8_t> h_fz_dist;
  sme::DevBuf d_bq_off;
  sme::DevBuf d_bq_docno;
  sme::DevBuf d_bq_score;
  int64_t bq_total = 0;
  uint64_t bq_cands = 0, bq_matches = 0;
  std::vector<int64_t> h_bq_off;
  std::vector<int32_t> h_bq_docno;
  std::vector<double> h_bq_score;
  sme::DevBuf d_ps_off;
  sme::DevBuf d_ps_terms;
  sme::DevBuf d_ps_docno;
  int64_t ps_records = 0, ps_terms = 0;
  bool has_positions = false;
  int64_t idf_N = 0;
  sme::DevBuf d_pq_off;
  sme::DevBuf d_pq_docno;
  sme::DevBuf d_pq_freq;
  sme::DevBuf d_pq_score;
  int64_t pq_total = 0;
  uint64_t pq_cands = 0, pq_verified = 0, pq_matches = 0;
  std::vector<int64_t> h_pq_off;
  std::vector<int32_t> h_pq_docno, h_pq_freq;
  std::vector<double> h_pq_score;
  std::vector<std::pair<std::string, float>> profile;
  ~sme_index() { ctx->live_indexes--; }
  explicit sme_index(sme_ctx *c) : ctx(c) {
    c->live_indexes++;
    for (sme::DevBuf *b : {&d_term_off, &d_term_chars, &d_off, &d_docno_d, &d_tf_d, &d_w, &d_idf, &d_lut, &d_gram, &d_docno_o,
                           &d_tf_o, &d_rec_docno, &d_rec_first, &d_ser, &d_hrow_of, &d_heavy, &d_spk, &d_wkeys, &d_wgoff,
                           &d_wgterm, &d_wx_off, &d_wx_ids, &d_wx_in, &d_wx_plan, &d_wx_choff, &d_wx_moff, &d_wx_scan, &d_fz_off,
                           &d_fz_ids, &d_fz_dist, &d_bq_off, &d_bq_docno, &d_bq_score, &d_ps_off, &d_ps_terms, &d_ps_docno,
                           &d_pq_off, &d_pq_docno, &d_pq_freq, &d_pq_score})
      b->pool = &c->pool;
  }
};

namespace sme {
struct Prof {
  hipStream_t st;
  std::vector<hipEvent_t> *pool;
  std::vector<std::pair<std::string, hipEvent_t>> ev;
  Prof(hipStream_t s, std::vector<hipEvent_t> *p) : st(s), pool(p) { mark("start"); }
  ~Prof() {
    for (auto &e : ev) pool->push_back(e.second);
  }
  void mark(const char *name) {
    hipEvent_t e;
    if (!pool->empty()) {
      e = pool->back();
      pool->pop_back();
    } else {
      SME_HIP(hipEventCreate(&e));
    }
    ev.emplace_back(name, e);
    last_stage() = name;
    SME_HIP(hipEventRecord(e, st));
  }
  std::vector<std::pair<std::string, float>> finish() {
    SME_HIP(hipEventSynchronize(ev.back().second));
    std::vector<std::pair<std::string, float>> out;
    for (size_t i = 1; i < ev.size(); i++) {
      float ms = 0;
      SME_HIP(hipEventElapsedTime(&ms, ev[i - 1].second, ev[i].second));
      out.emplace_back(ev[i].first, ms);
    }
    float tot = 0;
    SME_HIP(hipEventElapsedTime(&tot, ev.front().second, ev.back().second));
    out.emplace_back("total", tot);
    for (auto &p : ev) pool->push_back(p.second);
    ev.clear();
    return out;
  }
};

struct RecordSpans {
  uint64_t *rs, *re;
  int64_t nR;
  uint64_t *C;
  int64_t nC;
  int lt_attempts;
};
void build_docid_hash(sme_ctx *cx, bool distinct, hipStream_t st);
RecordSpans find_records(sme_ctx *cx, const uint8_t *d_text, uint64_t n, hipStream_t st, Prof *prof);
void split_points(sme_ctx *cx, const uint8_t *d_text, uint64_t n, int world, uint64_t *h_cuts, hipStream_t st);
void number_documents(sme_ctx *cx, const uint8_t *d_text, uint64_t n, hipStream_t st, std::vector<uint8_t> &out);
sme_index *build_index(sme_ctx *cx, const uint8_t *d_text, uint64_t n, hipStream_t st, int job = 0);
void chargram_stage(sme_ctx *cx, sme_index *ix, const int32_t *tstream, int64_t M, int64_t V, const int64_t *term_off,
                    const uint16_t *term_chars, hipStream_t st, Prof *prof);
uint32_t *term_sort(uint32_t *k0, uint32_t *v0, uint32_t *k1, uint32_t *v1, int64_t nrec, const int64_t *reg,
                    const int64_t *xoff, int64_t P, int bits, int64_t dmin, uint32_t F, int32_t *docno, int32_t *tf,
                    uint32_t *counts, hipStream_t st, const double *lut = nullptr, double idf = 0.0,
                    double *w = nullptr, int maxbits = 11, const uint2 *xw = nullptr, int64_t Pout = 0,
                    const uint32_t *rec_val = nullptr, int tf_shift = 0);
int term_sort_passes(int bits, int maxbits);
size_t term_sort_scratch(int64_t P);
template <typename K>
uint32_t *kv_sort(K *k0, uint32_t *v0, K *k1, uint32_t *v1, int64_t n, int bits, uint32_t *scratch, hipStream_t st,
                  bool keys_out = false);
size_t kv_sort_scratch(int64_t n);
template <typename T>
void excl_scan(const T *in, T *out, int64_t n, DevBuf &scratch, hipStream_t st);
void select_flagged(const uint8_t *flag, int64_t n, int32_t *out, int32_t *d_count, DevBuf &s1, DevBuf &s2,
                    hipStream_t st);
template <typename K>
void sort_pairs(K *keys_in, K *keys_out, uint32_t *vals_in, uint32_t *vals_out, int64_t n, int bits, DevBuf &radix,
                hipStream_t st);
template <typename K>
void sort_pairs_v64(K *keys_in, K *keys_out, const uint64_t *vals_in, uint64_t *vals_out, int64_t n, int bits,
                    DevBuf &ia, DevBuf &ib, DevBuf &radix, hipStream_t st);
template <typename T>
void reduce_max(const T *in, int64_t n, T *d_max, hipStream_t st);
void reduce_by_key_sum(const uint64_t *keys, const int32_t *vals, int64_t n, uint64_t *ukeys, int32_t *sums,
                       int64_t *d_runs, DevBuf &flags, DevBuf &pos, DevBuf &scan, hipStream_t st);
void serialize_index(sme_index *ix, hipStream_t st);
void pack_pieces(sme_index *ix, int world, uint8_t *d_out, uint64_t *sizes, hipStream_t st);
sme_index *merge_pieces(sme_ctx *cx, const uint8_t *d_blobs, const uint64_t *sizes, int np, hipStream_t st);
void reweight_index(sme_index *ix, int64_t N, const int64_t *d_gdf, hipStream_t st,
                    const uint32_t *d_term_of = nullptr);
sme_index *load_records(sme_ctx *cx, const uint8_t *d_records, const uint64_t *part_offsets, int np, hipStream_t st);
void prepare_queries(sme_index *ix, hipStream_t st);
void query_topk(sme_index *ix, const int32_t *d_terms, const int64_t *d_qoff, int nq, int k,
                int32_t *d_out_docno, double *d_out_score, uint32_t *d_out_tie, hipStream_t st, int tie_bits = 0);
void query_topk_java7(sme_index *ix, const int32_t *d_terms, const int64_t *d_qoff, int nq, int k,
                      int32_t *d_out_docno, double *d_out_score, uint32_t *d_out_tie, hipStream_t st);
void tokenize_string(sme_ctx *cx, const uint8_t *h_utf8, size_t n, std::vector<std::vector<uint16_t>> &out,
                     hipStream_t st);
void term_fingerprints(sme_index *ix, uint64_t *d_out, hipStream_t st);
void dfx_pack(sme_ctx *cx, const uint64_t *fp, const int64_t *df, int64_t n, int world, uint64_t *sfp, int64_t *sdf,
              int64_t *pos, int64_t *h_counts, hipStream_t st);
void dfx_sum(sme_ctx *cx, const uint64_t *fp, const int64_t *df, int64_t n, int64_t *out, int64_t *h_distinct,
             hipStream_t st);
void dfx_unpack(const int64_t *ret, const int64_t *pos, int64_t n, int64_t *out, hipStream_t st);
void merge_rows(const double *s, const int32_t *d, const uint32_t *t, int64_t rows, int m, int k, int32_t *od,
                double *os, uint32_t *ot, hipStream_t st);
int64_t count_shared_keys(sme_ctx *cx, const uint64_t *rows, int64_t n, hipStream_t st);
void lookup_terms(sme_index *ix, const std::vector<std::vector<uint16_t>> &terms, int32_t *ids,
                  hipStream_t st);
void prepare_wildcards(sme_index *ix, hipStream_t st);
void expand_wildcards(sme_index *ix, const uint8_t *patterns, const int64_t *offs, int n, hipStream_t st);
void suggest_terms(sme_index *ix, const uint8_t *words, const int64_t *offs, int n, int max_dist, int m,
                   hipStream_t st);
void query_boolean(sme_index *ix, const int32_t *term_ids, const int64_t *g_offsets, const uint8_t *g_flags,
                   const int64_t *q_offsets, int nq, int order, int m, hipStream_t st);
void query_phrase(sme_index *ix, const int32_t *term_ids, const int64_t *p_offsets, int np, int order, int m,
                  hipStream_t st);
inline double idf_value(int64_t N, int64_t df) { return log10((double)(N / df)); }
}
```

Measured before the change: 173.6.

## Restructure segmented tf sort with LDS-staged tile placement and global scan

Moves the per-term tf-descending sort into a separate tf_sort_segments routine. The large-segment path now stores tile histograms column-major and replaces the per-segment scan kernel with one global exclusive scan. Its placement kernel runs one tile per block and stages rows in LDS so global writes are coalesced. The count kernel uses vectorized int4 loads with a fast path for tf==1, and the wave and medium paths get new kernels. Several kernels now run on the aux stream, the tile-count readback goes through pinned memory, and tf_d must be 16-byte aligned.

```diff
diff --git a/simple-mapreduce-search-engine-information-retrieval-_amd/csrc/sme_build.hip b/simple-mapreduce-search-engine-information-retrieval-_amd/csrc/sme_build.hip
--- a/simple-mapreduce-search-engine-information-retrieval-_amd/csrc/sme_build.hip
+++ b/simple-mapreduce-search-engine-information-retrieval-_amd/csrc/sme_build.hip
@@ -2816,318 +2816,6 @@
     for (int c = 0; c < K; c++) gcomp[g * K + c] = tstream[(int64_t)rep[g] + c];
 }
 
-constexpr int kTfTiny = 8;
-constexpr int kTfSmall = 64;
-constexpr int kTfWave = 512;
-constexpr int kTfMedium = 8192;
-constexpr int kTfSortMaxTf = 1023;
-
-__global__ __launch_bounds__(256) void k_tfsort_tiny(const int64_t *__restrict__ off, int64_t V,
-                                                     const int32_t *__restrict__ docno_d,
-                                                     const int32_t *__restrict__ tf_d, int32_t *docno_o,
-                                                     int32_t *tf_o) {
-  for (int64_t s = blockIdx.x * (int64_t)blockDim.x + threadIdx.x; s < V; s += (int64_t)gridDim.x * blockDim.x) {
-    const int64_t b = off[s];
-    const int n = (int)(off[s + 1] - b);
-    if (n > kTfTiny || n == 0) continue;
-    int32_t t[kTfTiny], d[kTfTiny];
-#pragma unroll
-    for (int j = 0; j < kTfTiny; j++) {
-      t[j] = j < n ? tf_d[b + j] : INT_MIN;
-      d[j] = j < n ? docno_d[b + j] : 0;
-    }
-#pragma unroll
-    for (int j = 1; j < kTfTiny; j++) {
-#pragma unroll
-      for (int k = j; k > 0; k--) {
-        if (t[k - 1] < t[k]) {
-          const int32_t x = t[k - 1], y = d[k - 1];
-          t[k - 1] = t[k];
-          d[k - 1] = d[k];
-          t[k] = x;
-          d[k] = y;
-        }
-      }
-    }
-#pragma unroll
-    for (int j = 0; j < kTfTiny; j++)
-      if (j < n) {
-        docno_o[b + j] = d[j];
-        tf_o[b + j] = t[j];
-      }
-  }
-}
-
-__global__ __launch_bounds__(256) void k_tfsort_small(const int64_t *__restrict__ off,
-                                                      const int32_t *__restrict__ seg,
-                                                      const unsigned long long *__restrict__ nseg,
-                                                      const int32_t *__restrict__ docno_d,
-                                                      const int32_t *__restrict__ tf_d, int32_t *docno_o,
-                                                      int32_t *tf_o) {
-  const int lane = threadIdx.x & 63;
-  const int64_t nw = (int64_t)gridDim.x * (blockDim.x >> 6), ns = (int64_t)*nseg;
-  for (int64_t q = (int64_t)blockIdx.x * (blockDim.x >> 6) + (threadIdx.x >> 6); q < ns; q += nw) {
-    const int64_t s = seg[q];
-    const int64_t b = off[s];
-    const int n = (int)(off[s + 1] - b);
-    const bool v = lane < n;
-    const int32_t t = v ? tf_d[b + lane] : 0, d = v ? docno_d[b + lane] : 0;
-    int r = 0;
-    for (int j = 0; j < n; j++) {
-      const int32_t tj = __shfl(t, j, 64);
-      r += (tj > t) || (tj == t && j < lane);
-    }
-    if (v) {
-      docno_o[b + r] = d;
-      tf_o[b + r] = t;
-    }
-  }
-}
-
-template <int NW>
-__global__ __launch_bounds__(NW * 64) void k_tfsort_block(const int64_t *__restrict__ off, int64_t V,
-                                                          const int32_t *__restrict__ docno_d,
-                                                          const int32_t *__restrict__ tf_d, int32_t *docno_o,
-                                                          int32_t *tf_o, const int32_t *__restrict__ seg,
-                                                          const unsigned long long *__restrict__ nseg, int max_tf) {
-  extern __shared__ int32_t cnt[];
-  __shared__ int32_t wsum[NW];
-  constexpr int NT = NW * 64;
-  const int tid = threadIdx.x, w = tid >> 6, lane = tid & 63;
-  const int L = (max_tf + 1) * NW;
-  const uint64_t lt_mask = (1ull << lane) - 1;
-  const int64_t ns = (int64_t)*nseg;
-  for (int64_t q = blockIdx.x; q < ns; q += gridDim.x) {
-    const int64_t s = seg[q];
-    const int64_t b = off[s], n = off[s + 1] - b;
-    for (int j = tid; j < L; j += NT) cnt[j] = 0;
-    __syncthreads();
-    const int64_t nch = (n + 63) >> 6, cpw = (nch + NW - 1) / NW;
-    const int64_t c0 = (int64_t)w * cpw, c1 = c0 + cpw < nch ? c0 + cpw : nch;
-    int32_t tn = c0 < c1 && (c0 << 6) + lane < n ? tf_d[b + (c0 << 6) + lane] : -1;
-    for (int64_t c = c0; c < c1; c++) {
-      const int64_t i = (c << 6) + lane;
-      const bool v = i < n;
-      const int32_t t = tn;
-      tn = c + 1 < c1 && i + 64 < n ? tf_d[b + i + 64] : -1;
-      uint64_t pend = __ballot(v);
-      while (pend) {
-        const int32_t tv = __shfl(t, __ffsll((unsigned long long)pend) - 1, 64);
-        const uint64_t m = __ballot(t == tv);
-        if (lane == 0) cnt[(max_tf - tv) * NW + w] += __popcll(m);
-        pend &= ~m;
-      }
-    }
-    __syncthreads();
-    const int per = (L + NT - 1) / NT, j0 = tid * per, j1 = j0 + per < L ? j0 + per : L;
-    int run = 0;
-    for (int j = j0; j < j1; j++) run += cnt[j];
-    int inc = run;
-#pragma unroll
-    for (int o = 1; o < 64; o <<= 1) {
-      const int u = __shfl_up(inc, o, 64);
-      if (lane >= o) inc += u;
-    }
-    if (lane == 63) wsum[w] = inc;
-    __syncthreads();
-    int base = inc - run;
-    for (int k = 0; k < w; k++) base += wsum[k];
-    for (int j = j0; j < j1; j++) {
-      const int c = cnt[j];
-      cnt[j] = base;
-      base += c;
-    }
-    __syncthreads();
-    int32_t tn2 = -1, dn2 = 0;
-    if (c0 < c1 && (c0 << 6) + lane < n) {
-      tn2 = tf_d[b + (c0 << 6) + lane];
-      dn2 = docno_d[b + (c0 << 6) + lane];
-    }
-    for (int64_t c = c0; c < c1; c++) {
-      const int64_t i = (c << 6) + lane;
-      const bool v = i < n;
-      const int32_t t = tn2, d = dn2;
-      if (c + 1 < c1 && i + 64 < n) {
-        tn2 = tf_d[b + i + 64];
-        dn2 = docno_d[b + i + 64];
-      } else {
-        tn2 = -1;
-      }
-      uint64_t pend = __ballot(v);
-      while (pend) {
-        const int32_t tv = __shfl(t, __ffsll((unsigned long long)pend) - 1, 64);
-        const uint64_t m = __ballot(t == tv);
-        const int slot = (max_tf - tv) * NW + w;
-        const int cb = cnt[slot];
-        if (t == tv) {
-          const int64_t p = b + cb + __popcll(m & lt_mask);
-          docno_o[p] = d;
-          tf_o[p] = t;
-        }
-        if (lane == 0) cnt[slot] = cb + __popcll(m);
-        pend &= ~m;
-      }
-    }
-    __syncthreads();
-  }
-}
-
-constexpr int kTfTile = 4096;
-
-__global__ __launch_bounds__(256) void k_tf_classify(const int64_t *__restrict__ off, int64_t V, int32_t *med,
-                                                     int32_t *large, int32_t *small, int32_t *wave,
-                                                     unsigned long long *ctr) {
-  __shared__ unsigned int s_n[4];
-  __shared__ unsigned long long s_b[4];
-  for (int64_t s0 = (int64_t)blockIdx.x * 256; s0 < V; s0 += (int64_t)gridDim.x * 256) {
-    const int64_t s = s0 + threadIdx.x;
-    const int64_t n = s < V ? off[s + 1] - off[s] : 0;
-    const int cls = n > kTfMedium ? 1 : n > kTfWave ? 0 : n > kTfSmall ? 3 : n > kTfTiny ? 2 : -1;
-    if (threadIdx.x < 4) s_n[threadIdx.x] = 0;
-    __syncthreads();
-    unsigned int pos = 0;
-    if (cls >= 0) pos = atomicAdd(&s_n[cls], 1u);
-    __syncthreads();
-    if (threadIdx.x < 4)
-      s_b[threadIdx.x] = s_n[threadIdx.x] ? atomicAdd(&ctr[threadIdx.x], (unsigned long long)s_n[threadIdx.x]) : 0ull;
-    __syncthreads();
-    if (cls == 0) med[s_b[0] + pos] = (int32_t)s;
-    if (cls == 1) large[s_b[1] + pos] = (int32_t)s;
-    if (cls == 2) small[s_b[2] + pos] = (int32_t)s;
-    if (cls == 3) wave[s_b[3] + pos] = (int32_t)s;
-    __syncthreads();
-  }
-}
-__global__ void k_tf_ntiles(const int64_t *off, const int32_t *large, const unsigned long long *nlarge, int64_t V,
-                            int64_t *nt) {
-  const int64_t nl = (int64_t)*nlarge;
-  for (int64_t q = blockIdx.x * (int64_t)blockDim.x + threadIdx.x; q <= V; q += (int64_t)gridDim.x * blockDim.x) {
-    const int64_t n = q < nl ? off[large[q] + 1] - off[large[q]] : 0;
-    nt[q] = (n + kTfTile - 1) / kTfTile;
-  }
-}
-
-__device__ __forceinline__ int64_t tile_segment(const int64_t *toff, int64_t V, int64_t tau) {
-  int64_t lo = 0, hi = V;
-  while (hi - lo > 1) {
-    const int64_t mid = (lo + hi) >> 1;
-    if (toff[mid] <= tau) lo = mid;
-    else hi = mid;
-  }
-  return lo;
-}
-
-__global__ __launch_bounds__(256) void k_tf_tile_count(const int64_t *__restrict__ off,
-                                                       const int32_t *__restrict__ large,
-                                                       const unsigned long long *__restrict__ nlarge,
-                                                       const int64_t *__restrict__ toff, int64_t ntiles,
-                                                       const int32_t *__restrict__ tf_d, int max_tf,
-                                                       int32_t *tcnt) {
-  extern __shared__ int32_t h[];
-  const int w = threadIdx.x >> 6, lane = threadIdx.x & 63, F = max_tf + 1;
-  int32_t *hw = h + w * F;
-  const int64_t nwv = (int64_t)gridDim.x * 4;
-  const int64_t nl = (int64_t)*nlarge;
-  for (int64_t tau = (int64_t)blockIdx.x * 4 + w; tau < ntiles; tau += nwv) {
-    const int64_t q = tile_segment(toff, nl, tau), s = large[q];
-    const int64_t b = off[s] + (tau - toff[q]) * kTfTile, e = min(off[s + 1], b + (int64_t)kTfTile);
-    for (int j = lane; j < F; j += 64) hw[j] = 0;
-    __builtin_amdgcn_wave_barrier();
-    int32_t tn = b + lane < e ? tf_d[b + lane] : -1;
-    for (int64_t c = b; c < e; c += 64) {
-      const bool v = c + lane < e;
-      const int32_t t = tn;
-      tn = c + 64 + lane < e ? tf_d[c + 64 + lane] : -1;
-      uint64_t pend = __ballot(v);
-      while (pend) {
-        const int32_t tv = __shfl(t, __ffsll((unsigned long long)pend) - 1, 64);
-        const uint64_t m = __ballot(t == tv);
-        if (lane == 0) hw[max_tf - tv] += __popcll(m);
-        pend &= ~m;
-      }
-    }
-    __builtin_amdgcn_wave_barrier();
-    for (int j = lane; j < F; j += 64) tcnt[tau * F + j] = hw[j];
-    __builtin_amdgcn_wave_barrier();
-  }
-}
-
-__global__ __launch_bounds__(256) void k_tf_tile_scan(const unsigned long long *__restrict__ nlarge,
-                                                      const int64_t *__restrict__ toff, int max_tf, int32_t *tcnt) {
-  __shared__ int32_t sc[256 / 64 + 1];
-  const int tid = threadIdx.x, F = max_tf + 1;
-  const int64_t nl = (int64_t)*nlarge;
-  for (int64_t q = blockIdx.x; q < nl; q += gridDim.x) {
-    const int64_t t0 = toff[q], T = toff[q + 1] - t0;
-    int32_t *c = tcnt + t0 * F;
-    int32_t carry = 0;
-    for (int f0 = 0; f0 < F; f0 += 256) {
-      const int f = f0 + tid;
-      int32_t tot = 0;
-      if (f < F) {
-#pragma unroll 8
-        for (int64_t j = 0; j < T; j++) tot += c[j * F + f];
-      }
-      int32_t all;
-      int32_t run = carry + block_excl_sum<256, int32_t>(tot, sc, &all);
-      carry += all;
-      if (f < F) {
-#pragma unroll 8
-        for (int64_t j = 0; j < T; j++) {
-          const int32_t x = c[j * F + f];
-          c[j * F + f] = run;
-          run += x;
-        }
-      }
-    }
-  }
-}
-
-__global__ __launch_bounds__(256) void k_tf_tile_place(const int64_t *__restrict__ off,
-                                                       const int32_t *__restrict__ large,
-                                                       const unsigned long long *__restrict__ nlarge,
-                                                       const int64_t *__restrict__ toff, int64_t ntiles,
-                                                       const int32_t *__restrict__ docno_d,
-                                                       const int32_t *__restrict__ tf_d, int max_tf,
-                                                       const int32_t *__restrict__ tcnt, int32_t *docno_o,
-                                                       int32_t *tf_o) {
-  extern __shared__ int32_t h[];
-  const int w = threadIdx.x >> 6, lane = threadIdx.x & 63, F = max_tf + 1;
-  int32_t *hw = h + w * F;
-  const uint64_t lt_mask = (1ull << lane) - 1;
-  const int64_t nwv = (int64_t)gridDim.x * 4;
-  const int64_t nl = (int64_t)*nlarge;
-  for (int64_t tau = (int64_t)blockIdx.x * 4 + w; tau < ntiles; tau += nwv) {
-    const int64_t q = tile_segment(toff, nl, tau), s = large[q];
-    const int64_t sb = off[s];
-    const int64_t b = sb + (tau - toff[q]) * kTfTile, e = min(off[s + 1], b + (int64_t)kTfTile);
-    for (int j = lane; j < F; j += 64) hw[j] = tcnt[tau * F + j];
-    __builtin_amdgcn_wave_barrier();
-    int32_t tn = b + lane < e ? tf_d[b + lane] : -1, dnx = b + lane < e ? docno_d[b + lane] : 0;
-    for (int64_t c = b; c < e; c += 64) {
-      const bool v = c + lane < e;
-      const int32_t t = tn, d = dnx;
-      const int64_t in = c + 64 + lane;
-      tn = in < e ? tf_d[in] : -1;
-      dnx = in < e ? docno_d[in] : 0;
-      uint64_t pend = __ballot(v);
-      while (pend) {
-        const int32_t tv = __shfl(t, __ffsll((unsigned long long)pend) - 1, 64);
-        const uint64_t m = __ballot(t == tv);
-        const int slot = max_tf - tv;
-        const int cb = hw[slot];
-        if (t == tv) {
-          const int64_t p = sb + cb + __popcll(m & lt_mask);
-          docno_o[p] = d;
-          tf_o[p] = t;
-        }
-        if (lane == 0) hw[slot] = cb + __popcll(m);
-        pend &= ~m;
-      }
-    }
-    __builtin_amdgcn_wave_barrier();
-  }
-}
 
 static int grid_for(int64_t n, int nt = 256, int cap = 8192) {
   int64_t g = (n + nt - 1) / nt;
@@ -4211,49 +3899,8 @@
 
   int32_t *docno_o = ix->d_docno_o.as<int32_t>(PP + 1), *tf_o = ix->d_tf_o.as<int32_t>(PP + 1);
   if (PP > 0 && max_tf <= kTfSortMaxTf) {
-    hipLaunchKernelGGL(k_tfsort_tiny, dim3(grid_for(Vi)), dim3(256), 0, st, off, Vi, docno_d, tf_d, docno_o, tf_o);
-    int64_t *ntl = W[W_FKEYS].as<int64_t>(3 * (Vi + 1)), *toff = W[W_FREPS].as<int64_t>(Vi + 1);
-    int32_t *seg_med = reinterpret_cast<int32_t *>(ntl + Vi + 1), *seg_large = seg_med + Vi,
-            *seg_small = seg_large + Vi, *seg_wave = seg_small + Vi;
-    unsigned long long *nseg = cnt + 28;
-    SME_HIP(hipMemsetAsync(nseg, 0, 4 * sizeof(unsigned long long), st));
-    hipLaunchKernelGGL(k_tf_classify, dim3(grid_for(Vi)), dim3(256), 0, st, off, Vi, seg_med, seg_large, seg_small,
-                       seg_wave, nseg);
-    hipStream_t s2 = cx->aux_stream;
-    SME_HIP(hipEventRecord(cx->ev_fork, st));
-    SME_HIP(hipStreamWaitEvent(s2, cx->ev_fork, 0));
-    struct AuxJoin {
-      hipStream_t st, s2;
-      hipEvent_t ev;
-      ~AuxJoin() {
-        (void)hipEventRecord(ev, s2);
-        (void)hipStreamWaitEvent(st, ev, 0);
-      }
-    } aux_join{st, s2, cx->ev_join};
-    hipLaunchKernelGGL(k_tfsort_small, dim3(grid_for(Vi * 64, 256, 8192)), dim3(256), 0, s2, off, seg_small, nseg + 2,
-                       docno_d, tf_d, docno_o, tf_o);
-    const size_t lds4 = (size_t)(max_tf + 1) * 4 * sizeof(int32_t);
-    hipLaunchKernelGGL(k_tfsort_block<4>, dim3((unsigned)std::min<int64_t>(std::max<int64_t>(Vi, 1), 4096)),
-                       dim3(256), lds4, s2, off, Vi, docno_d, tf_d, docno_o, tf_o, seg_med, nseg, max_tf);
-    hipLaunchKernelGGL(k_tfsort_block<1>, dim3((unsigned)std::min<int64_t>(std::max<int64_t>(Vi, 1), 32768)),
-                       dim3(64), lds4 / 4, s2, off, Vi, docno_d, tf_d, docno_o, tf_o, seg_wave, nseg + 3, max_tf);
-    SME_CHECK_LAUNCH();
-    hipLaunchKernelGGL(k_tf_ntiles, dim3(grid_for(Vi + 1)), dim3(256), 0, st, off, seg_large, nseg + 1, Vi, ntl);
-    size_t tbb = 0;
-    excl_scan(ntl, toff, (int64_t)(Vi + 1), cx->ws[23], st);
-    const int64_t ntiles = d2h(toff + Vi, st);
-    if (ntiles > 0) {
-      const int F = max_tf + 1;
-      int32_t *tcnt = reinterpret_cast<int32_t *>(W[W_CKEY].as<uint64_t>((ntiles * F + 1) / 2 + 1));
-      const unsigned tg = (unsigned)std::min<int64_t>((ntiles + 3) / 4, 8192);
-      hipLaunchKernelGGL(k_tf_tile_count, dim3(tg), dim3(256), (size_t)4 * F * sizeof(int32_t), st, off, seg_large,
-                         nseg + 1, toff, ntiles, tf_d, max_tf, tcnt);
-      hipLaunchKernelGGL(k_tf_tile_scan, dim3((unsigned)std::min<int64_t>(Vi, 8192)), dim3(256), 0, st, nseg + 1,
-                         toff, max_tf, tcnt);
-      hipLaunchKernelGGL(k_tf_tile_place, dim3(tg), dim3(256), (size_t)4 * F * sizeof(int32_t), st, off, seg_large,
-                         nseg + 1, toff, ntiles, docno_d, tf_d, max_tf, tcnt, docno_o, tf_o);
-    }
-    SME_CHECK_LAUNCH();
+    tf_sort_segments(off, Vi, PP, docno_d, tf_d, max_tf, docno_o, tf_o, W[W_FKEYS], W[W_FREPS], W[W_CKEY], cx->ws[23],
+                     cnt + 28, st, cx->aux_stream, cx->ev_fork, cx->ev_join);
   } else if (PP > 0) {
     const int tfb = bits_for((uint64_t)max_tf);
     const int kbits = bits_for((uint64_t)std::max<int64_t>(Vi, 1));
diff --git a/simple-mapreduce-search-engine-information-retrieval-_amd/csrc/sme_internal.hpp b/simple-mapreduce-search-engine-information-retrieval-_amd/csrc/sme_internal.hpp
--- a/simple-mapreduce-search-engine-information-retrieval-_amd/csrc/sme_internal.hpp
+++ b/simple-mapreduce-search-engine-information-retrieval-_amd/csrc/sme_internal.hpp
@@ -256,6 +256,11 @@
 void reduce_max(const T *in, int64_t n, T *d_max, hipStream_t st);
 void reduce_by_key_sum(const uint64_t *keys, const int32_t *vals, int64_t n, uint64_t *ukeys, int32_t *sums,
                        int64_t *d_runs, DevBuf &flags, DevBuf &pos, DevBuf &scan, hipStream_t st);
+constexpr int kTfSortMaxTf = 1023;
+void tf_sort_segments(const int64_t *off, int64_t V, int64_t P, const int32_t *docno_d, const int32_t *tf_d,
+                      int max_tf, int32_t *docno_o, int32_t *tf_o, DevBuf &lists, DevBuf &tiles, DevBuf &tcnt, DevBuf &scan,
+                      unsigned long long *nseg, hipStream_t st, hipStream_t aux_stream, hipEvent_t ev_fork,
+                      hipEvent_t ev_join);
 void serialize_index(sme_index *ix, hipStream_t st);
 void pack_pieces(sme_index *ix, int world, uint8_t *d_out, uint64_t *sizes, hipStream_t st);
 sme_index *merge_pieces(sme_ctx *cx, const uint8_t *d_blobs, const uint64_t *sizes, int np, hipStream_t st);
diff --git a/simple-mapreduce-search-engine-information-retrieval-_amd/csrc/sme_tfsort.hip b/simple-mapreduce-search-engine-information-retrieval-_amd/csrc/sme_tfsort.hip
--- /dev/null
+++ b/simple-mapreduce-search-engine-information-retrieval-_amd/csrc/sme_tfsort.hip
@@ -0,0 +1,543 @@
+#include <hip/hip_runtime.h>
+#include <limits.h>
+#include <stdint.h>
+
+#include <algorithm>
+
+#include "sme_internal.hpp"
+
+namespace sme {
+namespace {
+
+constexpr int kTfTiny = 8;
+constexpr int kTfSmall = 64;
+constexpr int kTfWave = 512;
+constexpr int kTfMedium = 8192;
+constexpr int kTfTile = 4096;
+constexpr int kTfK = 8;
+constexpr int kTfK4 = 4;
+static_assert(kTfWave == kTfK * 64, "k_tfsort_wave holds a whole segment in kTfK chunks");
+
+int grid_for(int64_t n, int nt = 256, int cap = 8192) {
+  int64_t g = (n + nt - 1) / nt;
+  if (g < 1) g = 1;
+  if (g > cap) g = cap;
+  return (int)g;
+}
+
+__global__ __launch_bounds__(256) void k_tfsort_tiny(const int64_t *__restrict__ off, int64_t V,
+                                                     const int32_t *__restrict__ docno_d,
+                                                     const int32_t *__restrict__ tf_d, int32_t *docno_o,
+                                                     int32_t *tf_o) {
+  for (int64_t s = blockIdx.x * (int64_t)blockDim.x + threadIdx.x; s < V; s += (int64_t)gridDim.x * blockDim.x) {
+    const int64_t b = off[s];
+    const int n = (int)(off[s + 1] - b);
+    if (n > kTfTiny || n == 0) continue;
+    int32_t t[kTfTiny], d[kTfTiny];
+#pragma unroll
+    for (int j = 0; j < kTfTiny; j++) {
+      t[j] = j < n ? tf_d[b + j] : INT_MIN;
+      d[j] = j < n ? docno_d[b + j] : 0;
+    }
+#pragma unroll
+    for (int j = 1; j < kTfTiny; j++) {
+#pragma unroll
+      for (int k = j; k > 0; k--) {
+        if (t[k - 1] < t[k]) {
+          const int32_t x = t[k - 1], y = d[k - 1];
+          t[k - 1] = t[k];
+          d[k - 1] = d[k];
+          t[k] = x;
+          d[k] = y;
+        }
+      }
+    }
+#pragma unroll
+    for (int j = 0; j < kTfTiny; j++)
+      if (j < n) {
+        docno_o[b + j] = d[j];
+        tf_o[b + j] = t[j];
+      }
+  }
+}
+
+__device__ __forceinline__ int32_t lane_value(int32_t v, int l) { return __builtin_amdgcn_readlane(v, l); }
+__device__ __forceinline__ int first_lane(uint64_t m) { return __ffsll((unsigned long long)m) - 1; }
+
+template <int NW>
+__device__ __forceinline__ void count_chunk(int32_t t, bool v, int32_t *cnt, int w, int max_tf, int lane, int &c1) {
+  const uint64_t m1 = __ballot(v && t == 1);
+  c1 += __popcll(m1);
+  uint64_t pend = __ballot(v) & ~m1;
+  while (pend) {
+    const int32_t tv = lane_value(t, first_lane(pend));
+    const uint64_t m = __ballot(t == tv) & pend;
+    if (lane == 0) atomicAdd(&cnt[(max_tf - tv) * NW + w], __popcll(m));
+    pend &= ~m;
+  }
+}
+
+template <int NW>
+__device__ __forceinline__ void place_chunk(int32_t t, int32_t d, bool v, int32_t *cnt, int w, int max_tf, int lane,
+                                            uint64_t lt_mask, int &base1, int64_t sb, int32_t *docno_o,
+                                            int32_t *tf_o) {
+  const uint64_t m1 = __ballot(v && t == 1);
+  if (m1) {
+    if (m1 >> lane & 1) {
+      const int64_t p = sb + base1 + __popcll(m1 & lt_mask);
+      docno_o[p] = d;
+      tf_o[p] = t;
+    }
+    base1 += __popcll(m1);
+  }
+  uint64_t pend = __ballot(v) & ~m1;
+  while (pend) {
+    const int32_t tv = lane_value(t, first_lane(pend));
+    const uint64_t m = __ballot(t == tv) & pend;
+    const int slot = (max_tf - tv) * NW + w;
+    const int cb = cnt[slot];
+    if (m >> lane & 1) {
+      const int64_t p = sb + cb + __popcll(m & lt_mask);
+      docno_o[p] = d;
+      tf_o[p] = t;
+    }
+    if (lane == 0) cnt[slot] = cb + __popcll(m);
+    pend &= ~m;
+  }
+}
+
+struct SegWalk {
+  const int64_t *off;
+  const int32_t *seg;
+  int64_t ns, stride, q1, b, b1;
+  int64_t n, n1;
+  int32_t s2;
+  __device__ __forceinline__ bool start(const int64_t *off_, const int32_t *seg_, int64_t ns_, int64_t q0,
+                                        int64_t stride_) {
+    off = off_, seg = seg_, ns = ns_, stride = stride_;
+    if (q0 >= ns) return false;
+    const int64_t s = seg[q0];
+    b = off[s];
+    n = off[s + 1] - b;
+    q1 = q0 + stride;
+    b1 = 0, n1 = 0;
+    if (q1 < ns) {
+      const int64_t s1 = seg[q1];
+      b1 = off[s1];
+      n1 = off[s1 + 1] - b1;
+    }
+    s2 = q1 + stride < ns ? seg[q1 + stride] : 0;
+    return true;
+  }
+  int64_t b2, n2;
+  int32_t s3;
+  __device__ __forceinline__ void prefetch() {
+    b2 = 0, n2 = 0;
+    if (q1 + stride < ns) {
+      b2 = off[s2];
+      n2 = off[(int64_t)s2 + 1] - b2;
+    }
+    s3 = q1 + 2 * stride < ns ? seg[q1 + 2 * stride] : 0;
+  }
+  __device__ __forceinline__ bool advance() {
+    if (q1 >= ns) return false;
+    b = b1, n = n1;
+    b1 = b2, n1 = n2;
+    s2 = s3;
+    q1 += stride;
+    return true;
+  }
+};
+
+__global__ __launch_bounds__(256) void k_tfsort_small(const int64_t *__restrict__ off,
+                                                      const int32_t *__restrict__ seg,
+                                                      const unsigned long long *__restrict__ nseg,
+                                                      const int32_t *__restrict__ docno_d,
+                                                      const int32_t *__restrict__ tf_d, int32_t *docno_o,
+                                                      int32_t *tf_o) {
+  const int lane = threadIdx.x & 63;
+  const uint64_t lt_mask = (1ull << lane) - 1;
+  SegWalk sw;
+  if (!sw.start(off, seg, (int64_t)*nseg, (int64_t)blockIdx.x * (blockDim.x >> 6) + (threadIdx.x >> 6),
+                (int64_t)gridDim.x * (blockDim.x >> 6)))
+    return;
+  int32_t t = lane < sw.n ? tf_d[sw.b + lane] : -1, d = lane < sw.n ? docno_d[sw.b + lane] : 0;
+  for (;;) {
+    const int32_t tn = lane < sw.n1 ? tf_d[sw.b1 + lane] : -1, dn = lane < sw.n1 ? docno_d[sw.b1 + lane] : 0;
+    sw.prefetch();
+    const bool v = lane < sw.n;
+    const uint64_t vm = __ballot(v);
+    int r = 0;
+    uint64_t pend = vm;
+    while (pend) {
+      const int32_t tv = lane_value(t, first_lane(pend));
+      const uint64_t m = __ballot(t == tv) & pend;
+      r += t < tv ? __popcll(m) : t == tv ? __popcll(m & lt_mask) : 0;
+      pend &= ~m;
+    }
+    if (v) {
+      docno_o[sw.b + r] = d;
+      tf_o[sw.b + r] = t;
+    }
+    if (!sw.advance()) break;
+    t = tn, d = dn;
+  }
+}
+
+__global__ __launch_bounds__(256) void k_tfsort_wave(const int64_t *__restrict__ off,
+                                                     const int32_t *__restrict__ seg,
+                                                     const unsigned long long *__restrict__ nseg,
+                                                     const int32_t *__restrict__ docno_d,
+                                                     const int32_t *__restrict__ tf_d, int max_tf, int32_t *docno_o,
+                                                     int32_t *tf_o) {
+  extern __shared__ int32_t cnt[];
+  const int w = threadIdx.x >> 6, lane = threadIdx.x & 63, F = max_tf + 1;
+  int32_t *hw = cnt + w * F;
+  int32_t *sd = cnt + 4 * F + w * 2 * kTfWave, *stf = sd + kTfWave;
+  const uint64_t lt_mask = (1ull << lane) - 1;
+  SegWalk sw;
+  if (!sw.start(off, seg, (int64_t)*nseg, (int64_t)blockIdx.x * 4 + w, (int64_t)gridDim.x * 4)) return;
+  do {
+    const int64_t b = sw.b;
+    const int n = (int)sw.n;
+    int32_t t[kTfK], d[kTfK];
+#pragma unroll
+    for (int k = 0; k < kTfK; k++) t[k] = k * 64 + lane < n ? tf_d[b + k * 64 + lane] : -1;
+#pragma unroll
+    for (int k = 0; k < kTfK; k++) d[k] = k * 64 + lane < n ? docno_d[b + k * 64 + lane] : 0;
+    sw.prefetch();
+    for (int j = lane; j < F; j += 64) hw[j] = 0;
+    __builtin_amdgcn_wave_barrier();
+    int c1 = 0;
+#pragma unroll
+    for (int k = 0; k < kTfK; k++)
+      if (k * 64 < n) count_chunk<1>(t[k], k * 64 + lane < n, hw, 0, max_tf, lane, c1);
+    if (lane == 0) atomicAdd(&hw[max_tf - 1], c1);
+    __builtin_amdgcn_wave_barrier();
+    int carry = 0;
+    for (int j0 = 0; j0 < F; j0 += 64) {
+      const int j = j0 + lane;
+      const int x = j < F ? hw[j] : 0;
+      const int inc = wave_incl_sum(x);
+      if (j < F) hw[j] = carry + inc - x;
+      carry += lane_value(inc, 63);
+    }
+    __builtin_amdgcn_wave_barrier();
+    int base1 = __builtin_amdgcn_readfirstlane(hw[max_tf - 1]);
+#pragma unroll
+    for (int k = 0; k < kTfK; k++)
+      if (k * 64 < n)
+        place_chunk<1>(t[k], d[k], k * 64 + lane < n, hw, 0, max_tf, lane, lt_mask, base1, 0, sd, stf);
+    __builtin_amdgcn_wave_barrier();
+#pragma unroll
+    for (int k = 0; k < kTfK; k++)
+      if (k * 64 + lane < n) {
+        docno_o[b + k * 64 + lane] = sd[k * 64 + lane];
+        tf_o[b + k * 64 + lane] = stf[k * 64 + lane];
+      }
+    __builtin_amdgcn_wave_barrier();
+  } while (sw.advance());
+}
+
+__device__ __forceinline__ void block_scan_counters(int32_t *cnt, int L, int32_t *wsum) {
+  const int tid = threadIdx.x, w = tid >> 6, lane = tid & 63;
+  const int per = (L + 255) / 256, j0 = tid * per, j1 = j0 + per < L ? j0 + per : L;
+  int run = 0;
+  for (int j = j0; j < j1; j++) run += cnt[j];
+  const int inc = wave_incl_sum(run);
+  if (lane == 63) wsum[w] = inc;
+  __syncthreads();
+  int base = inc - run;
+  for (int k = 0; k < w; k++) base += wsum[k];
+  for (int j = j0; j < j1; j++) {
+    const int c = cnt[j];
+    cnt[j] = base;
+    base += c;
+  }
+}
+
+__global__ __launch_bounds__(256) void k_tfsort_medium(const int64_t *__restrict__ off,
+                                                       const int32_t *__restrict__ seg,
+                                                       const unsigned long long *__restrict__ nseg,
+                                                       const int32_t *__restrict__ docno_d,
+                                                       const int32_t *__restrict__ tf_d, int max_tf,
+                                                       int32_t *docno_o, int32_t *tf_o) {
+  extern __shared__ int32_t cnt[];
+  constexpr int NW = 4, NT = NW * 64;
+  __shared__ int32_t wsum[NW];
+  const int tid = threadIdx.x, w = tid >> 6, lane = tid & 63;
+  const int L = (max_tf + 1) * NW;
+  const uint64_t lt_mask = (1ull << lane) - 1;
+  SegWalk sw;
+  if (!sw.start(off, seg, (int64_t)*nseg, blockIdx.x, gridDim.x)) return;
+  do {
+    const int64_t b = sw.b;
+    const int n = (int)sw.n;
+    const int nch = (n + 63) >> 6, cpw = (nch + NW - 1) / NW;
+    const int c0 = w * cpw, c1 = c0 + cpw < nch ? c0 + cpw : nch;
+    int32_t t[kTfK], d[kTfK];
+#pragma unroll
+    for (int k = 0; k < kTfK; k++) {
+      const int i = (c0 + k) * 64 + lane;
+      t[k] = c0 + k < c1 && i < n ? tf_d[b + i] : -1;
+    }
+    sw.prefetch();
+    for (int j = tid; j < L; j += NT) cnt[j] = 0;
+    __syncthreads();
+    int ones = 0;
+    for (int cb = c0; cb < c1; cb += kTfK) {
+      if (cb != c0) {
+#pragma unroll
+        for (int k = 0; k < kTfK; k++) {
+          const int i = (cb + k) * 64 + lane;
+          t[k] = cb + k < c1 && i < n ? tf_d[b + i] : -1;
+        }
+      }
+#pragma unroll
+      for (int k = 0; k < kTfK; k++)
+        if (cb + k < c1) count_chunk<NW>(t[k], (cb + k) * 64 + lane < n, cnt, w, max_tf, lane, ones);
+    }
+    if (lane == 0) atomicAdd(&cnt[(max_tf - 1) * NW + w], ones);
+    __syncthreads();
+    block_scan_counters(cnt, L, wsum);
+    __syncthreads();
+    int base1 = __builtin_amdgcn_readfirstlane(cnt[(max_tf - 1) * NW + w]);
+    for (int cb = c0; cb < c1; cb += kTfK) {
+#pragma unroll
+      for (int k = 0; k < kTfK; k++) {
+        const int i = (cb + k) * 64 + lane;
+        t[k] = cb + k < c1 && i < n ? tf_d[b + i] : -1;
+      }
+#pragma unroll
+      for (int k = 0; k < kTfK; k++) {
+        const int i = (cb + k) * 64 + lane;
+        d[k] = cb + k < c1 && i < n ? docno_d[b + i] : 0;
+      }
+#pragma unroll
+      for (int k = 0; k < kTfK; k++)
+        if (cb + k < c1)
+          place_chunk<NW>(t[k], d[k], (cb + k) * 64 + lane < n, cnt, w, max_tf, lane, lt_mask, base1, b, docno_o,
+                          tf_o);
+    }
+    __syncthreads();
+  } while (sw.advance());
+}
+
+__global__ __launch_bounds__(256) void k_tf_classify(const int64_t *__restrict__ off, int64_t V, int32_t *med,
+                                                     int32_t *large, int32_t *small, int32_t *wave,
+                                                     unsigned long long *ctr) {
+  __shared__ unsigned int s_n[4];
+  __shared__ unsigned long long s_b[4];
+  for (int64_t s0 = (int64_t)blockIdx.x * 256; s0 < V; s0 += (int64_t)gridDim.x * 256) {
+    const int64_t s = s0 + threadIdx.x;
+    const int64_t n = s < V ? off[s + 1] - off[s] : 0;
+    const int cls = n > kTfMedium ? 1 : n > kTfWave ? 0 : n > kTfSmall ? 3 : n > kTfTiny ? 2 : -1;
+    if (threadIdx.x < 4) s_n[threadIdx.x] = 0;
+    __syncthreads();
+    unsigned int pos = 0;
+    if (cls >= 0) pos = atomicAdd(&s_n[cls], 1u);
+    __syncthreads();
+    if (threadIdx.x < 4)
+      s_b[threadIdx.x] = s_n[threadIdx.x] ? atomicAdd(&ctr[threadIdx.x], (unsigned long long)s_n[threadIdx.x]) : 0ull;
+    __syncthreads();
+    if (cls == 0) med[s_b[0] + pos] = (int32_t)s;
+    if (cls == 1) large[s_b[1] + pos] = (int32_t)s;
+    if (cls == 2) small[s_b[2] + pos] = (int32_t)s;
+    if (cls == 3) wave[s_b[3] + pos] = (int32_t)s;
+    __syncthreads();
+  }
+}
+
+
+__global__ void k_tf_ntiles(const int64_t *off, const int32_t *large, const unsigned long long *nlarge,
+                            int64_t nlmax, int64_t *nt) {
+  const int64_t nl = (int64_t)*nlarge;
+  for (int64_t q = blockIdx.x * (int64_t)blockDim.x + threadIdx.x; q <= nlmax; q += (int64_t)gridDim.x * blockDim.x) {
+    const int64_t n = q < nl ? off[large[q] + 1] - off[large[q]] : 0;
+    nt[q] = (n + kTfTile - 1) / kTfTile;
+  }
+}
+
+__device__ __forceinline__ int64_t tile_segment(const int64_t *toff, int64_t V, int64_t tau) {
+  int64_t lo = 0, hi = V;
+  while (hi - lo > 1) {
+    const int64_t mid = (lo + hi) >> 1;
+    if (toff[mid] <= tau) lo = mid;
+    else hi = mid;
+  }
+  return lo;
+}
+
+__device__ __forceinline__ int4 load_tf4(const int32_t *__restrict__ tf_d, int64_t i, int64_t b, int64_t e) {
+  if (i >= b && i + 4 <= e) return *reinterpret_cast<const int4 *>(tf_d + i);
+  int4 r;
+  r.x = i >= b && i < e ? tf_d[i] : -1;
+  r.y = i + 1 >= b && i + 1 < e ? tf_d[i + 1] : -1;
+  r.z = i + 2 >= b && i + 2 < e ? tf_d[i + 2] : -1;
+  r.w = i + 3 >= b && i + 3 < e ? tf_d[i + 3] : -1;
+  return r;
+}
+
+__global__ __launch_bounds__(256) void k_tf_tile_count(const int64_t *__restrict__ off,
+                                                       const int32_t *__restrict__ large,
+                                                       const unsigned long long *__restrict__ nlarge,
+                                                       const int64_t *__restrict__ toff, int64_t ntiles,
+                                                       const int32_t *__restrict__ tf_d, int max_tf,
+                                                       uint32_t *tcnt, int32_t *tile_q) {
+  extern __shared__ int32_t h[];
+  const int w = threadIdx.x >> 6, lane = threadIdx.x & 63, F = max_tf + 1;
+  int32_t *hw = h + w * F;
+  const int64_t nwv = (int64_t)gridDim.x * 4;
+  const int64_t nl = (int64_t)*nlarge;
+  for (int64_t tau = (int64_t)blockIdx.x * 4 + w; tau < ntiles; tau += nwv) {
+    const int64_t q = tile_segment(toff, nl, tau), s = large[q];
+    const int64_t t0 = toff[q], T = toff[q + 1] - t0;
+    const int64_t b = off[s] + (tau - t0) * kTfTile, e = min(off[s + 1], b + (int64_t)kTfTile);
+    const int64_t a0 = b & ~(int64_t)3;
+    const int ng = (int)((e - a0 + 3) >> 2);
+    if (lane == 0) tile_q[tau] = (int32_t)q;
+    for (int j = lane; j < F; j += 64) hw[j] = 0;
+    __builtin_amdgcn_wave_barrier();
+    int c1 = 0;
+    for (int g0 = 0; g0 < ng; g0 += 64 * kTfK4) {
+      int4 x[kTfK4];
+#pragma unroll
+      for (int k = 0; k < kTfK4; k++) {
+        const int g = g0 + k * 64 + lane;
+        x[k] = g < ng ? load_tf4(tf_d, a0 + 4 * (int64_t)g, b, e) : make_int4(-1, -1, -1, -1);
+      }
+#pragma unroll
+      for (int k = 0; k < kTfK4; k++)
+        if (g0 + k * 64 < ng) {
+          count_chunk<1>(x[k].x, x[k].x >= 0, hw, 0, max_tf, lane, c1);
+          count_chunk<1>(x[k].y, x[k].y >= 0, hw, 0, max_tf, lane, c1);
+          count_chunk<1>(x[k].z, x[k].z >= 0, hw, 0, max_tf, lane, c1);
+          count_chunk<1>(x[k].w, x[k].w >= 0, hw, 0, max_tf, lane, c1);
+        }
+    }
+    if (lane == 0) atomicAdd(&hw[max_tf - 1], c1);
+    __builtin_amdgcn_wave_barrier();
+    uint32_t *col = tcnt + t0 * F + (tau - t0);
+    for (int j = lane; j < F; j += 64) col[(int64_t)j * T] = (uint32_t)hw[j];
+    __builtin_amdgcn_wave_barrier();
+  }
+}
+
+constexpr int kTfQ = kTfTile / 4 / 64;
+static_assert(kTfQ * 4 * 64 == kTfTile, "four waves hold a whole tile");
+__global__ __launch_bounds__(256, 4) void k_tf_tile_place(const int64_t *__restrict__ off,
+                                                       const int32_t *__restrict__ large,
+                                                       const int32_t *__restrict__ tile_q,
+                                                       const int64_t *__restrict__ toff, int64_t ntiles,
+                                                       const int32_t *__restrict__ docno_d,
+                                                       const int32_t *__restrict__ tf_d, int max_tf,
+                                                       const uint32_t *__restrict__ tcnt, int32_t *docno_o,
+                                                       int32_t *tf_o) {
+  extern __shared__ int32_t h[];
+  __shared__ int32_t wsum[4];
+  const int tid = threadIdx.x, w = tid >> 6, lane = tid & 63, F = max_tf + 1;
+  int32_t *delta = h, *cnt = h + F, *sd = h + 5 * F, *stf = sd + kTfTile;
+  const uint64_t lt_mask = (1ull << lane) - 1;
+  for (int64_t tau = blockIdx.x; tau < ntiles; tau += gridDim.x) {
+    const int64_t q = tile_q[tau], s = large[q];
+    const int64_t t0 = toff[q], T = toff[q + 1] - t0;
+    const int64_t sb = off[s];
+    const int64_t b = sb + (tau - t0) * kTfTile;
+    const int n = (int)(min(off[s + 1], b + (int64_t)kTfTile) - b);
+    const int i0 = w * (kTfQ * 64) + lane;
+    int32_t t[kTfQ], d[kTfQ];
+#pragma unroll
+    for (int k = 0; k < kTfQ; k++) t[k] = i0 + k * 64 < n ? tf_d[b + i0 + k * 64] : -1;
+#pragma unroll
+    for (int k = 0; k < kTfQ; k++) d[k] = i0 + k * 64 < n ? docno_d[b + i0 + k * 64] : 0;
+    const uint32_t *col = tcnt + t0 * F + (tau - t0);
+    const uint32_t seg0 = tcnt[t0 * F];
+    for (int j = tid; j < F; j += 256) delta[j] = (int32_t)(col[(int64_t)j * T] - seg0);
+    for (int j = tid; j < 4 * F; j += 256) cnt[j] = 0;
+    __syncthreads();
+    int ones = 0;
+#pragma unroll
+    for (int k = 0; k < kTfQ; k++)
+      if (w * (kTfQ * 64) + k * 64 < n) count_chunk<4>(t[k], i0 + k * 64 < n, cnt, w, max_tf, lane, ones);
+    if (lane == 0) atomicAdd(&cnt[(max_tf - 1) * 4 + w], ones);
+    __syncthreads();
+    block_scan_counters(cnt, 4 * F, wsum);
+    __syncthreads();
+    for (int j = tid; j < F; j += 256) delta[j] -= cnt[j * 4];
+    int base1 = __builtin_amdgcn_readfirstlane(cnt[(max_tf - 1) * 4 + w]);
+    __syncthreads();
+#pragma unroll
+    for (int k = 0; k < kTfQ; k++)
+      if (w * (kTfQ * 64) + k * 64 < n)
+        place_chunk<4>(t[k], d[k], i0 + k * 64 < n, cnt, w, max_tf, lane, lt_mask, base1, 0, sd, stf);
+    __syncthreads();
+    for (int p = tid; p < n; p += 256) {
+      const int32_t tv = stf[p];
+      const int64_t g = sb + delta[max_tf - tv] + p;
+      docno_o[g] = sd[p];
+      tf_o[g] = tv;
+    }
+    __syncthreads();
+  }
+}
+
+}
+
+void tf_sort_segments(const int64_t *off, int64_t V, int64_t P, const int32_t *docno_d, const int32_t *tf_d,
+                      int max_tf, int32_t *docno_o, int32_t *tf_o, DevBuf &lists, DevBuf &tiles, DevBuf &tcnt_buf, DevBuf &scan,
+                      unsigned long long *nseg, hipStream_t st, hipStream_t aux_stream, hipEvent_t ev_fork,
+                      hipEvent_t ev_join) {
+  if (max_tf < 1 || max_tf > kTfSortMaxTf || (reinterpret_cast<uintptr_t>(tf_d) & 15))
+    throw Error(SME_EINVAL, "tf_sort_segments: max_tf outside 1.." + std::to_string(kTfSortMaxTf) +
+                                " or tf_d not 16-byte aligned");
+  if (V <= 0 || P <= 0) return;
+  int64_t *ntl = lists.as<int64_t>(3 * (V + 1)), *toff = tiles.as<int64_t>(V + 1);
+  int32_t *seg_med = reinterpret_cast<int32_t *>(ntl + V + 1), *seg_large = seg_med + V, *seg_small = seg_large + V,
+          *seg_wave = seg_small + V;
+  SME_HIP(hipMemsetAsync(nseg, 0, 4 * sizeof(unsigned long long), st));
+  hipLaunchKernelGGL(k_tf_classify, dim3(grid_for(V)), dim3(256), 0, st, off, V, seg_med, seg_large, seg_small,
+                     seg_wave, nseg);
+  SME_HIP(hipEventRecord(ev_fork, st));
+  SME_HIP(hipStreamWaitEvent(aux_stream, ev_fork, 0));
+  struct AuxJoin {
+    hipStream_t st, s2;
+    hipEvent_t ev;
+    ~AuxJoin() {
+      (void)hipEventRecord(ev, s2);
+      (void)hipStreamWaitEvent(st, ev, 0);
+    }
+  } aux_join{st, aux_stream, ev_join};
+  const int F = max_tf + 1;
+  const size_t lds4 = (size_t)4 * F * sizeof(int32_t);
+  hipLaunchKernelGGL(k_tfsort_small, dim3(grid_for(V * 64, 256, 8192)), dim3(256), 0, aux_stream, off, seg_small,
+                     nseg + 2, docno_d, tf_d, docno_o, tf_o);
+  hipLaunchKernelGGL(k_tfsort_medium, dim3((unsigned)std::min<int64_t>(V, 4096)), dim3(256), lds4, aux_stream, off,
+                     seg_med, nseg, docno_d, tf_d, max_tf, docno_o, tf_o);
+  hipLaunchKernelGGL(k_tfsort_wave, dim3(grid_for(V * 64, 256, 8192)), dim3(256),
+                     lds4 + (size_t)4 * 2 * kTfWave * sizeof(int32_t), aux_stream, off, seg_wave, nseg + 3, docno_d, tf_d,
+                     max_tf, docno_o, tf_o);
+  hipLaunchKernelGGL(k_tfsort_tiny, dim3(grid_for(V)), dim3(256), 0, aux_stream, off, V, docno_d, tf_d, docno_o, tf_o);
+  SME_CHECK_LAUNCH();
+  const int64_t nlmax = std::min<int64_t>(V, P / (kTfMedium + 1));
+  hipLaunchKernelGGL(k_tf_ntiles, dim3(grid_for(nlmax + 1)), dim3(256), 0, st, off, seg_large, nseg + 1, nlmax, ntl);
+  excl_scan(ntl, toff, nlmax + 1, scan, st);
+  static thread_local int64_t *pin = nullptr;
+  if (!pin) SME_HIP(hipHostMalloc(reinterpret_cast<void **>(&pin), 64, hipHostMallocDefault));
+  SME_HIP(hipMemcpyAsync(pin, toff + nlmax, sizeof(int64_t), hipMemcpyDeviceToHost, st));
+  SME_HIP(hipStreamSynchronize(st));
+  const int64_t ntiles = *pin;
+  if (ntiles > 0) {
+    uint32_t *tcnt = tcnt_buf.as<uint32_t>((size_t)ntiles * F + 2 + (size_t)ntiles);
+    int32_t *tile_q = reinterpret_cast<int32_t *>(tcnt + (size_t)ntiles * F + 2);
+    const unsigned tg = (unsigned)std::min<int64_t>((ntiles + 3) / 4, 8192);
+    hipLaunchKernelGGL(k_tf_tile_count, dim3(tg), dim3(256), lds4, st, off, seg_large, nseg + 1, toff, ntiles, tf_d,
+                       max_tf, tcnt, tile_q);
+    excl_scan(tcnt, tcnt, ntiles * F, scan, st);
+    hipLaunchKernelGGL(k_tf_tile_place, dim3((unsigned)std::min<int64_t>(ntiles, 16384)), dim3(256),
+                       (size_t)(5 * F + 2 * kTfTile) * sizeof(int32_t), st, off, seg_large, (const int32_t *)tile_q, toff,
+                       ntiles, docno_d, tf_d, max_tf, tcnt, docno_o, tf_o);
+  }
+  SME_CHECK_LAUNCH();
+}
+
+}
```

After: 178.1, median of 6. 2.6% higher.
